# troyvvgroup/quemb

Measured on AMD Instinct MI355X. Metric: fragment CCSD iters/sec (full BE sweep over synthetic n_occ=20 n_virt=200 fragments); corr-E error vs oracle in parity_max_abs_err_Eh / parity_n220_abs_err_Eh, higher is better.
Workload: dtype f64

## Files before the change

### include/qemb_hip_ops.h

```cpp
#ifndef QEMB_HIP_OPS_H
#define QEMB_HIP_OPS_H
#include "qemb_hip.h"
#ifdef __cplusplus
extern "C" {
#endif

#define QEMB_TIMER_LADDER 0
#define QEMB_TIMER_RINGS 1
#define QEMB_TIMER_ITER 2
#define QEMB_TIMER_AO2MO 3
#define QEMB_TIMER_SCF 4
#define QEMB_TIMER_GEMM_ANY 5
#define QEMB_TIMER_SCHMIDT 6
#define QEMB_TIMER_DF 7
int qemb_timer_begin(int slot);
int qemb_timer_end(int slot);
int qemb_timer_read(int slot, double* total_ms, int64_t* count);
int qemb_timer_reset(int slot);
int qemb_alloc_stats(long long* n_driver_allocs, long long* n_driver_frees, double* ms_in_driver_calls, double* gb_allocated, int reset);
int qemb_gemm_flop_count(double* flops, int reset);
int qemb_tape_cache_counters(int64_t* reused, int64_t* recorded, int reset);
int qemb_ctx_timer_read(int ctx, int slot, double* total_ms, int64_t* count, int reset);
int qemb_timer_live_events(int slot);


int qemb_op_gemm(int64_t M, int64_t N, int64_t K, double alpha, const double* A, int64_t lda, int a_kcontig,
                 int64_t strideA, const double* B, int64_t ldb, int b_kcontig, int64_t strideB, double beta,
                 double* C, int64_t ldc, int64_t strideC, int64_t batch);
int qemb_op_gemm_slab_rows(int64_t M, int64_t N, int64_t K, const double* A, int64_t lda, int64_t a_slab, int64_t a_slab_skip, const double* B, int64_t ldb,
                           int b_kcontig, double* C, int64_t ldc, int cfg);
int qemb_set_gemm_config(int cfg);
int qemb_mfma_f64_peak(int iters, int blocks_per_cu, double* tflops);
int qemb_set_gemm_splitk(int enabled);
int qemb_op_gemm_probe(int64_t M, int64_t N, int64_t K, const double* A, int64_t lda, int a_kcontig, const double* B, int64_t ldb, int b_kcontig,
                       double* C, int64_t ldc, int cfg, int ksplit, double* ms, double* clock_ghz, int64_t* workgroups);
int qemb_op_gemm_stamps(int64_t M, int64_t N, int64_t K, const double* A, int64_t lda, const double* B, int64_t ldb, double* C, int64_t ldc, int cfg,
                        int ksplit, double* out7);
int qemb_pair_gemm_choice(int64_t rows, int64_t cols, int* cfg, int* ksplit);
int qemb_set_gemm_ksplit(int ksplit);
int qemb_op_copy4(const int64_t dim[4], const double* in, const int64_t si[4], double* out,
                  const int64_t so[4], double alpha, double beta);
int qemb_op_outer4(const int64_t dim[4], const double* u, int64_t su0, int64_t su2, const double* v,
                   int64_t sv1, int64_t sv3, double* out, const int64_t so[4], double alpha, double beta);
int qemb_op_div_denom(double* x, int64_t d0, int64_t d1, int64_t d2, int64_t d3, const double* ea,
                      const double* eb, const double* ec, const double* ed);
int qemb_op_ladder_pack_vvvv(int64_t n, int64_t o, const double* M, double* Vp, int64_t ldp, double* Vm, int64_t ldm);
int qemb_op_ladder_pack_tau(int64_t o, int64_t v, const double* tau, double* Tp, int64_t ldp, double* Tm, int64_t ldm);
int qemb_op_ladder_scatter_pm(int64_t o, int64_t v, const double* Rp, int64_t ldp, const double* Rm, int64_t ldm, double* t2);
int qemb_op_dot(int64_t n, const double* x, const double* y, double* out_dev);
int qemb_op_absmax(int64_t n, const double* x, double* out_dev);
int qemb_op_gemv_rows(int64_t rows, int64_t cols, const double* T, int64_t ldt, const double* x, double* y,
                      double alpha, double beta);
int qemb_op_gemv_rows_batched(int64_t rows, int64_t cols, int64_t nbatch, const double* T, int64_t ldt, int64_t strideT,
                              const double* x, int64_t stridex, double* y, double alpha, double beta);
int qemb_op_contract_mid(int64_t outer, int64_t mid, int64_t inner, const double* T, const double* x,
                         double* Y, int64_t ldy, double alpha, double beta);
int qemb_op_unpack_s4(int64_t n, const double* s4, double* s1);
int qemb_op_pack_s4(int64_t n, const double* s1, double* s4);
int qemb_op_unpack_s8_to_s4(int64_t n, const double* s8, double* s4);
int qemb_op_mirror_lower(int64_t n, double* A, int64_t lda);
int qemb_op_k_from_pairs(int64_t n, const double* H, const double* D, double* K);
int qemb_op_jk_from_packed(int64_t n, const double* S4, const double* D, const double* Dp, double* Jp, double* K);
int qemb_op_pack_pm_cols(int64_t rows, int64_t v, const double* in, double* Op, int64_t ldp, double* Om, int64_t ldm);
int qemb_op_scatter_pm_rows(int64_t o, int64_t ncols, const double* Xp, const double* Xm, double* out);
int qemb_op_pack_w_pm(int64_t o, const double* W, double* Ap, int64_t lda_p, double* Am, int64_t lda_m);
int qemb_op_ladder_scatter_pm2(int64_t o, int64_t v, const double* Rp, int64_t ldp, const double* Rm, int64_t ldm, const double* Hp, const double* Hm,
                               int assign, double* t2);
int qemb_op_lincomb2(int64_t n, double a, const double* x, double b, const double* y, double beta, double* out);
int qemb_op_small_k_update(int64_t batch, int64_t M, int64_t N, int64_t K, double alpha, const double* A, int64_t sA, const double* B, int64_t sB, double* C, int64_t sC);
int qemb_op_ccsd_ph_layouts(int64_t o, int64_t v, const double* t2, const double* t1, double* T, double* Tp, double* S, double* Ut, double* Tpt, double* Th);
int qemb_op_ccsd_y_traces(int64_t o, int64_t v, const double* ZC, const double* ZB, double* Y);
int qemb_op_copy4_two(const int64_t dim[4], const double* in, const int64_t si[4], double* out, const int64_t so[4], double alpha, double beta, const double* base,
                      double* out2, const double* in2, double c2a, double c2b);
int qemb_op_scatter_pm_rows_add(int64_t o, int64_t ncols, const double* Xp, const double* Xm, double* out, const double* add);
int qemb_op_ccsd_y_traces_add(int64_t o, int64_t v, const double* ZC, const double* ZB, double* Y, const double* add);
int qemb_op_pack_w_pm_sum(int64_t o, const double* Wt, const double* X, const double* At, double* Ap, int64_t lda_p, double* Am, int64_t lda_m);
int qemb_op_ccsd_t1_small(int64_t o, int64_t v, const double* t1, const double* Lvv, const double* Loo, const double* Fov, double* t1n);
int qemb_op_ccsd_t1_assemble(int64_t o, int64_t v, const double* t1, const double* Lvv, const double* Loo, const double* Fov, const double* S, const double* Lph1,
                             const double* PA, int SA, int64_t strideA, const double* PB, int SB, int64_t strideB, double* t1n);
int qemb_op_gemv_rows_two(int64_t rows1, int64_t cols1, const double* T1, int64_t ld1, const double* x1, double* y1, double a1, double b1,
                          int64_t rows2, int64_t cols2, const double* T2, int64_t ld2, const double* x2, double* y2, double a2, double b2);
int qemb_op_ccsd_y_traces_slabs(int64_t o, int64_t v, const double* ZC, const double* ZB, double* Y, const double* add, int S, int64_t stride, double scale);
int qemb_op_gemv_rows2(int64_t rows, int64_t cols, const double* T1, int64_t ld1, const double* x1, const double* T2, int64_t ld2, const double* x2, double* y, double alpha, double beta);
int qemb_op_ccsd_finish_t2_rings(int64_t o, int64_t v, double* t2n, const double* U, const double* OV, const double* RS, const double* M, const double* eo, const double* ev, double* t1n);
int qemb_op_diis_push(int64_t n, const double* trial, const double* prev, double* e, double* xcopy, int m, const double* const* ys, int self, double* row_dev, double* row_host);
int qemb_op_ccsd_extrapolate_energy(int64_t o, int64_t v, int nterms, const double* coef, const double* const* xs, double* amp, const double* L, double* tau, double* e_host);
int qemb_op_gather_rows(int64_t nrows, int64_t len, const int64_t* idx_dev, const double* src, int64_t ld, double* dst);
int qemb_op_scale_rows(int64_t nrows, int64_t len, double* x, const double* s);
int qemb_op_pack_pair_rows(int64_t n, int64_t ncols, const double* in, double* out);
int qemb_op_unpack_tril_pair_rows(int64_t nr, int64_t n, const double* in, double* full);
int qemb_op_extract_pf(int64_t n, const double* Mp, int64_t p0, int64_t q0, int64_t r0, int64_t s0, int64_t sp, int64_t sq,
                       int64_t sr, int64_t ss, double* out);
int qemb_op_extract_pf_t(int64_t n, const double* T, int64_t x0, int64_t r0, int64_t s0, int64_t c0, int64_t sx, int64_t sr,
                         int64_t ss, int64_t sc, double* out);
int qemb_op_ladder_pack_vvvv_pf(int64_t n, int64_t o, const double* Mp, double* Vp, int64_t ldp, double* Vm, int64_t ldm);
int qemb_op_unpack_tril_rows(int64_t rows, int64_t n, const double* packed, double* full);
int qemb_op_pack_tril_rows(int64_t rows, int64_t n, const double* full, double* packed);
int qemb_op_jacobi_eigh(int64_t n, double* A, double* w, double* V, int* sweeps);
int qemb_op_scf_fused_max(void);
int qemb_op_jacobi_eigh_in_basis(int64_t n, const double* F, const double* Cp, double* w, double* C_out, double* C2_out, int nocc, double* dm_out, double stop_below, int* sweeps);
int qemb_op_scf_fock_small(int64_t n, const double* h, const double* J, const double* K, const double* D, double* F, double* err, double* scal2);
int qemb_op_pack_density_sym(int64_t n, const double* D, double* Dp);
int qemb_op_jacobi_svd(int64_t m, int64_t n, double* G, double* s, double* U, double* V, int* sweeps);
int qemb_op_cholesky_lower(int64_t n, double* A);
int qemb_op_tri_inverse_lower(int64_t n, const double* L, double* Linv);


int qemb_op_mp2_amplitudes(int64_t o, int64_t v, const double* ovov, const double* eo, const double* ev, double* t2, double* G, double* e_host);

int qemb_op_rdm2_assemble(int kind, int64_t o, int64_t v, const double* t1, const double* t2, const double* dm1c, double* out);
int qemb_op_rdm2_add_nc(int64_t m, const double* g, double alpha, double* X);
int qemb_op_rdm2_symmetrize(int64_t m, const double* g, double* X);
int qemb_op_rdm2_eri_dot(int64_t m, int sym, const double* eri, const double* K, double* e_host);

int qemb_op_kdf_split(int64_t rows, int64_t nao, const double* z, double* planes);
int qemb_op_kdf_stack(int64_t nk, int64_t nao, int64_t n, const double* ta, double* Cs, double* Dk);
int qemb_op_kdf_pack(int64_t naux, int64_t n, const double* M, int paired, double w, double* F, int64_t ldf, double* out2_host);

int qemb_frag_prepare_ccsd(qemb_frag_t f, int nsocc, const double* h, const double* dm0, const qemb_solver_opts* opts);
int qemb_frag_ccsd_iterate(qemb_frag_t f, int niter, double* e_corr, double* normt);
int qemb_frag_ccsd_reset(qemb_frag_t f);
int qemb_frag_ccsd_export(qemb_frag_t f, const char* name, double* host, int64_t nelem);


int qemb_op_boys(int m_max, int64_t n, const double* x, double* out);
int qemb_op_int3c_class(int la, int lb, int lP, const void* bf_a, const void* bf_b, const void* bf_P, const double* c2s, double* out_host);
int qemb_op_int4c_class(int la, int lb, int lc, int ld, const void* bf_a, const void* bf_b, const void* bf_c, const void* bf_d, const double* c2s, double* out_host);
int qemb_op_int4c_tile(void* basis, const int32_t* pairs_r, int64_t n_r, const int32_t* pairs_s, int64_t n_s, double thresh, double* out_host);
int qemb_op_cd_panel_factor(int n, const double* A_host, double thr, double* T_host, int32_t* piv_host, int32_t* rank, int* in_lds);
int qemb_op_cd_diag_update(int64_t np, int r, const double* Lnew_host, const int32_t* pivrow_host, double* d_host, int64_t nsp, const int32_t* row0_host, const int32_t* cnt_host,
                           double* spmax_host, double* dmax_host);
int qemb_op_cd_permute(int64_t M, int64_t N, const double* L_host, const int32_t* pos_host, int full, double* out_host);
int qemb_op_df_get_ints(void* df, double* out_host, int* identity_metric);

int qemb_op_fci_sigma(int n, int nsocc, const double* h_host, const double* V_dev, const double* c_dev, double* sigma_dev);
int qemb_op_fci_rdm12(int n, int nsocc, const double* c_dev, int cumulant, double* dm1_host, double* dm2_dev);
int qemb_op_fci_sigma_timed(int n, int nsocc, const double* h_host, const double* V_dev, const double* c_dev, double* sigma_dev, double* ms3);
int qemb_op_fci_links(int n, int nsocc, int64_t* ns, int* nlink, int32_t* strings_host, int32_t* links_host);

#ifdef __cplusplus
}
#endif
#endif
```

### quemb_amd/_lib.py

```python

from __future__ import annotations

import ctypes as C
import os
from pathlib import Path

import numpy as np

_HERE = Path(__file__).resolve().parent
LIB_PATH = _HERE / "libqemb_hip.so"

c_dp = C.POINTER(C.c_double)
c_i64 = C.c_int64
c_vp = C.c_void_p


QEMB_ERR_ARG, QEMB_ERR_ALLOC, QEMB_ERR_DEVICE, QEMB_ERR_NOCONV, QEMB_ERR_NUMERIC, QEMB_ERR_UNSUPPORTED = -1, -2, -3, -4, -5, -6


class QembError(RuntimeError):

    def __init__(self, msg="", status=None):
        super().__init__(msg)
        self.status = status


class SolverOpts(C.Structure):
    _fields_ = [("struct_size", C.c_uint32), ("cc_conv_tol", C.c_double), ("cc_conv_tol_normt", C.c_double), ("cc_max_cycle", C.c_int),
                ("cc_diis_space", C.c_int), ("scf_conv_tol", C.c_double), ("scf_conv_tol_grad", C.c_double),
                ("scf_max_cycle", C.c_int), ("scf_diis_space", C.c_int), ("warm_start", C.c_int), ("verbose", C.c_int),
                ("relax_density", C.c_int), ("lambda_conv_tol", C.c_double), ("lambda_max_cycle", C.c_int),
                ("strict_convergence", C.c_int)]


class FciOpts(C.Structure):
    _fields_ = [("struct_size", C.c_uint32), ("conv_tol", C.c_double), ("max_cycle", C.c_int), ("max_space", C.c_int), ("lindep", C.c_double)]


_lib = None
_initialised_device = None


def _declare(lib):
    def f(name, restype, *argtypes):
        fn = getattr(lib, name)
        fn.restype = restype
        fn.argtypes = list(argtypes)

    I, D, P, V, L = C.c_int, C.c_double, c_vp, c_vp, c_i64
    f("qemb_init", I, I)
    f("qemb_last_error", C.c_char_p)
    f("qemb_backend", C.c_char_p)
    f("qemb_sync", I)
    f("qemb_device_sync", I)
    f("qemb_mem_info", I, C.POINTER(C.c_size_t), C.POINTER(C.c_size_t))
    f("qemb_malloc", I, C.POINTER(c_vp), C.c_size_t)
    f("qemb_free", I, V)
    f("qemb_trim", I)
    f("qemb_trim_all", I)
    f("qemb_h2d", I, V, V, C.c_size_t)
    f("qemb_d2h", I, V, V, C.c_size_t)
    f("qemb_h2d_async", I, V, V, C.c_size_t)
    f("qemb_d2d", I, V, V, C.c_size_t)
    f("qemb_timer_begin", I, I)
    f("qemb_timer_end", I, I)
    f("qemb_timer_read", I, I, C.POINTER(D), C.POINTER(L))
    f("qemb_timer_reset", I, I)
    f("qemb_timer_live_events", I, I)
    f("qemb_op_gemm", I, L, L, L, D, P, L, I, L, P, L, I, L, D, P, L, L, L)
    f("qemb_op_gemm_slab_rows", I, L, L, L, P, L, L, L, P, L, I, P, L, I)
    f("qemb_op_gemm_probe", I, L, L, L, P, L, I, P, L, I, P, L, I, I, C.POINTER(D), C.POINTER(D), C.POINTER(L))
    f("qemb_op_gemm_stamps", I, L, L, L, P, L, P, L, P, L, I, I, C.POINTER(D))
    f("qemb_set_gemm_config", I, I)
    f("qemb_set_gemm_splitk", I, I)
    f("qemb_set_gemm_ksplit", I, I)
    f("qemb_pair_gemm_choice", I, L, L, C.POINTER(I), C.POINTER(I))
    f("qemb_op_ladder_pack_vvvv", I, L, L, P, P, L, P, L)
    f("qemb_op_ladder_pack_tau", I, L, L, P, P, L, P, L)
    f("qemb_op_ladder_scatter_pm", I, L, L, P, L, P, L, P)
    f("qemb_mfma_f64_peak", I, I, I, C.POINTER(D))
    f("qemb_op_copy4", I, C.POINTER(L), P, C.POINTER(L), P, C.POINTER(L), D, D)
    f("qemb_op_outer4", I, C.POINTER(L), P, L, L, P, L, L, P, C.POINTER(L), D, D)
    f("qemb_op_div_denom", I, P, L, L, L, L, P, P, P, P)
    f("qemb_op_dot", I, L, P, P, P)
    f("qemb_op_mp2_amplitudes", I, L, L, P, P, P, P, P, C.POINTER(D))
    f("qemb_op_rdm2_assemble", I, I, L, L, P, P, P, P)
    f("qemb_op_rdm2_add_nc", I, L, P, D, P)
    f("qemb_op_rdm2_symmetrize", I, L, P, P)
    f("qemb_op_rdm2_eri_dot", I, L, I, P, P, C.POINTER(D))
    f("qemb_op_absmax", I, L, P, P)
    f("qemb_op_gemv_rows", I, L, L, P, L, P, P, D, D)
    f("qemb_op_gemv_rows_batched", I, L, L, L, P, L, L, P, L, P, D, D)
    f("qemb_op_contract_mid", I, L, L, L, P, P, P, L, D, D)
    f("qemb_op_unpack_s4", I, L, P, P)
    f("qemb_op_pack_s4", I, L, P, P)
    f("qemb_op_unpack_s8_to_s4", I, L, P, P)
    f("qemb_op_unpack_tril_rows", I, L, L, P, P)
    f("qemb_op_pack_pair_rows", I, L, L, P, P)
    f("qemb_op_mirror_lower", I, L, P, L)
    f("qemb_op_k_from_pairs", I, L, P, P, P)
    f("qemb_op_jk_from_packed", I, L, P, P, P, P, P)
    f("qemb_op_pack_pm_cols", I, L, L, P, P, L, P, L)
    f("qemb_op_scatter_pm_rows", I, L, L, P, P, P)
    f("qemb_op_pack_w_pm", I, L, P, P, L, P, L)
    f("qemb_op_ladder_scatter_pm2", I, L, L, P, L, P, L, P, P, I, P)
    f("qemb_op_lincomb2", I, L, D, P, D, P, D, P)
    f("qemb_op_small_k_update", I, L, L, L, L, D, P, L, P, L, P, L)
    f("qemb_op_ccsd_ph_layouts", I, L, L, P, P, P, P, P, P, P, P)
    f("qemb_op_ccsd_y_traces", I, L, L, P, P, P)
    f("qemb_op_copy4_two", I, C.POINTER(L), P, C.POINTER(L), P, C.POINTER(L), D, D, P, P, P, D, D)
    f("qemb_op_scatter_pm_rows_add", I, L, L, P, P, P, P)
    f("qemb_op_ccsd_y_traces_add", I, L, L, P, P, P, P)
    f("qemb_op_pack_w_pm_sum", I, L, P, P, P, P, L, P, L)
    f("qemb_op_ccsd_t1_small", I, L, L, P, P, P, P, P)
    f("qemb_op_gemv_rows2", I, L, L, P, L, P, P, L, P, P, D, D)
    f("qemb_op_ccsd_t1_assemble", I, L, L, P, P, P, P, P, P, P, I, L, P, I, L, P)
    f("qemb_op_gemv_rows_two", I, L, L, P, L, P, P, D, D, L, L, P, L, P, P, D, D)
    f("qemb_op_ccsd_y_traces_slabs", I, L, L, P, P, P, P, I, L, D)
    f("qemb_op_ccsd_finish_t2_rings", I, L, L, P, P, P, P, P, P, P, P)
    f("qemb_op_diis_push", I, L, P, P, P, P, I, P, I, P, P)
    f("qemb_op_ccsd_extrapolate_energy", I, L, L, I, P, P, P, P, P, P)
    f("qemb_op_gather_rows", I, L, L, P, P, L, P)
    f("qemb_op_scale_rows", I, L, L, P, P)
    f("qemb_ctx_count", I, I)
    f("qemb_ctx_bind", I, I)
    f("qemb_ctx_partition", I, I)
    f("qemb_ctx_timer_read", I, I, I, C.POINTER(C.c_double), C.POINTER(c_i64), I)
    f("qemb_gemm_flop_count", I, C.POINTER(C.c_double), I)
    f("qemb_tape_cache_counters", I, C.POINTER(L), C.POINTER(L), I)
    f("qemb_alloc_stats", I, C.POINTER(C.c_longlong), C.POINTER(C.c_longlong), C.POINTER(C.c_double), C.POINTER(C.c_double), I)
    f("qemb_op_unpack_tril_pair_rows", I, L, L, P, P)
    f("qemb_op_extract_pf", I, L, P, L, L, L, L, L, L, L, L, P)
    f("qemb_op_extract_pf_t", I, L, P, L, L, L, L, L, L, L, L, P)
    f("qemb_op_ladder_pack_vvvv_pf", I, L, L, P, P, L, P, L)
    f("qemb_op_pack_tril_rows", I, L, L, P, P)
    f("qemb_op_jacobi_eigh", I, L, P, P, P, C.POINTER(I))
    f("qemb_op_scf_fused_max", I)
    f("qemb_op_jacobi_eigh_in_basis", I, L, P, P, P, P, P, I, P, D, C.POINTER(I))
    f("qemb_op_scf_fock_small", I, L, P, P, P, P, P, P, P)
    f("qemb_op_pack_density_sym", I, L, P, P)
    f("qemb_op_jacobi_svd", I, L, L, P, P, P, P, C.POINTER(I))
    f("qemb_op_cholesky_lower", I, L, P)
    f("qemb_op_tri_inverse_lower", I, L, P, P)
    f("qemb_comm_unique_id", I, P)
    f("qemb_comm_init", I, I, I, P)
    f("qemb_comm_info", I, C.POINTER(I), C.POINTER(I))
    f("qemb_comm_allreduce", I, P, L, I)
    f("qemb_comm_destroy", I)
    OP = C.POINTER(SolverOpts)
    IP = C.POINTER(I)
    DP = C.POINTER(D)
    f("qemb_default_opts", None, OP)
    f("qemb_frag_create", I, I, I, C.POINTER(c_vp))
    f("qemb_frag_free", I, V)
    f("qemb_frag_set_eri_s4", I, V, P)
    f("qemb_frag_set_eri_s4_dev", I, V, P)
    f("qemb_frag_set_df_factor", I, V, I, P)
    f("qemb_frag_set_df_factor_dev", I, V, I, P)
    f("qemb_frag_mo_route", I, V, I)
    f("qemb_frag_set_df_only", I, V, I, P)
    f("qemb_frag_set_df_only_dev", I, V, I, V)
    f("qemb_frag_resident_bytes", I, V, C.POINTER(L))
    f("qemb_frag_mo_route_used", I, V, IP, IP)
    f("qemb_frag_get_eri_s4", I, V, P)
    f("qemb_frag_set_energy_data", I, V, P, P, P, D, IP, I)
    f("qemb_frag_jk", I, V, P, P, P)
    f("qemb_frag_solve", I, V, I, P, P, OP, I, P, P, P, P, P, P, P, DP, DP, DP, IP, IP)
    f("qemb_frag_solve_mp2", I, V, I, P, P, OP, I, P, P, P, P, P, P, DP, DP, DP, IP)
    f("qemb_frag_solve_mp2_batch", I, I, P, IP, P, P, OP, I, P, P, P, P, P, P, P, P, P, IP)
    f("qemb_default_fci_opts", None, C.POINTER(FciOpts))
    f("qemb_frag_solve_fci", I, V, I, P, P, OP, C.POINTER(FciOpts), I, P, P, P, P, P, P, DP, DP, DP, IP, IP)
    f("qemb_frag_fci_bytes", I, I, I, I, C.POINTER(L))
    f("qemb_frag_fci_mem_limit", I, V, L)
    f("qemb_frag_fci_residual", I, V, DP)
    f("qemb_op_fci_sigma", I, I, I, P, P, P, P)
    f("qemb_op_fci_rdm12", I, I, I, P, I, P, P)
    f("qemb_op_fci_sigma_timed", I, I, I, P, P, P, P, P)
    f("qemb_op_fci_links", I, I, I, C.POINTER(L), IP, P, P)
    f("qemb_frag_rdm2", I, V, I, I, P)
    f("qemb_frag_rdm2_mem_limit", I, V, L)
    f("qemb_frag_rdm2_dev", I, V, I, I, P)
    f("qemb_rdm2_full_guard", I, L, L, L)
    f("qemb_frag_lambda_iters", I, P, C.POINTER(C.c_int))
    f("qemb_frag_solve_batch", I, I, P, IP, P, P, OP, I, P, P, P, P, P, P, P, P, P, P, IP, IP, C.POINTER(L))
    f("qemb_frag_scf", I, V, I, P, P, OP, P, P, P, P, DP, IP, IP)
    f("qemb_frag_cphf", I, V, I, P, P, OP, P, I, P)
    f("qemb_ccsd_solve", I, I, I, I, P, P, P, OP, P, P, D, IP, I, P, P, P, P, P, P, DP, IP)
    f("qemb_frag_prepare_ccsd", I, V, I, P, P, OP)
    f("qemb_frag_ccsd_iterate", I, V, I, DP, DP)
    f("qemb_frag_ccsd_reset", I, V)
    f("qemb_frag_ccsd_export", I, V, C.c_char_p, P, L)
    LP = C.POINTER(L)
    f("qemb_aoeri_upload", I, I, P, I, C.POINTER(c_vp))
    f("qemb_aoeri_free", I, V)
    f("qemb_ao2mo_dense", I, V, P, I, P, V)
    f("qemb_df_create", I, I, P, C.POINTER(c_vp))
    f("qemb_lpq_upload", I, P, I, C.POINTER(c_vp))
    f("qemb_df_create_pbc", I, I, P, C.POINTER(c_vp), IP)
    f("qemb_df_alloc_ints", I, V, I)
    f("qemb_df_add_pw_block", I, V, I, P, P, P, P)
    f("qemb_df_add_rs_block", I, V, I, I, P)
    f("qemb_df_pw_imag_absmax", I, V, C.POINTER(C.c_double))
    f("qemb_df_pw_select", I, V, I)
    f("qemb_df_free", I, V)
    f("qemb_df_set_ints", I, V, I, P, I)
    f("qemb_df_set_ints_semisparse", I, V, I, L, P, P, P, P)
    f("qemb_df_transform", I, V, P, I, P, V)
    f("qemb_df_transform_screened", I, V, P, I, P, D, P, V)
    f("qemb_df_transform_factor", I, V, P, I, V)
    f("qemb_df_transform_screened_factor", I, V, P, I, P, D, V)
    f("qemb_kdf_create", I, I, I, I, IP, IP, C.POINTER(c_vp))
    f("qemb_kdf_set_pair", I, V, I, I, P)
    f("qemb_kdf_transform", I, V, P, I, P, V, I)
    f("qemb_kdf_free", I, V)
    f("qemb_kdf_guard", I, I, I, I, I, I, I, L)
    f("qemb_frag_get_df_factor", I, V, P)
    f("qemb_int_basis_create", I, I, P, C.c_size_t, P, C.POINTER(c_vp))
    f("qemb_int_basis_free", I, V)
    f("qemb_int3c2e", I, V, V, P, L, I, P, I)
    f("qemb_int2c2e", I, V, P, I)
    f("qemb_df_create_empty", I, C.POINTER(c_vp))
    f("qemb_df_set_ints_from_basis", I, V, V, V)
    f("qemb_df_set_ints_semisparse_from_basis", I, V, V, V, L, P, P, P, P)
    f("qemb_int4c2e", I, V, I, D, P, I)
    f("qemb_int4c_mem_limit", I, V, L)
    f("qemb_int4c_stats", I, V, C.POINTER(L), C.POINTER(L))
    f("qemb_aoeri_from_basis", I, V, D, C.POINTER(c_vp))
    f("qemb_int_jk_direct", I, V, P, D, P, P, I)
    f("qemb_int_jk_direct_bytes", I, V, C.POINTER(L))
    f("qemb_ao2mo_direct", I, V, I, P, P, P, P, L, D)
    f("qemb_ao2mo_direct_bytes", I, V, I, P, L, C.POINTER(L))
    f("qemb_int4c_tile_stats", I, V, C.POINTER(L), C.POINTER(L))
    f("qemb_op_int4c_tile", I, V, P, L, P, L, D, P)
    f("qemb_int_cholesky", I, V, D, D, L, L, P, C.POINTER(L))
    f("qemb_int_cholesky_bytes", I, V, L, L, C.POINTER(L))
    f("qemb_int_cholesky_stats", I, V, P)
    f("qemb_df_set_ints_from_cholesky", I, V, V, D, D, L, L)
    f("qemb_op_cd_panel_factor", I, I, P, D, P, P, C.POINTER(C.c_int32), C.POINTER(I))
    f("qemb_op_cd_diag_update", I, L, I, P, P, P, L, P, P, P, P)
    f("qemb_op_cd_permute", I, L, L, P, P, I, P)
    f("qemb_op_df_get_ints", I, V, P, C.POINTER(I))
    f("qemb_op_int4c_class", I, I, I, I, I, P, P, P, P, P, P)
    f("qemb_op_boys", I, I, L, P, P)
    f("qemb_op_int3c_class", I, I, I, I, P, P, P, P, P)
    f("qemb_op_kdf_split", I, L, L, P, P)
    f("qemb_op_kdf_stack", I, L, L, L, P, P, P)
    f("qemb_op_kdf_pack", I, L, L, P, I, D, P, L, DP)
    f("qemb_schmidt", I, P, I, I, I, LP, I, D, P, I, IP, IP)
    f("qemb_schmidt_subspace", I, P, I, I, I, LP, I, D, P, I, IP, IP)
    f("qemb_schmidt_svd", I, P, I, LP, I, D, P, I, IP, IP)
    f("qemb_nsocc_guess", I, P, I, I, P, IP, P)
    f("qemb_matmul", I, L, L, L, P, I, P, I, P)
    f("qemb_abs_overlap_prim", I, I, P, P, P, P, L, I, P, P, P)
    return lib


def load(path: os.PathLike | None = None):
    global _lib
    if _lib is None:
        p = Path(path) if path else LIB_PATH
        if not p.exists():
            raise QembError(
                f"{p} not found: build it with `python -c 'import __graft_entry__ as g; g.build()'` "
                "(make -C quemb_amd/csrc). quemb_amd has no CPU fallback."
            )
        _lib = _declare(C.CDLL(str(p)))
    return _lib


def declare(cdll):
    return _declare(cdll)


class ConvergenceWarning(RuntimeWarning):
    """A fragment solve did not converge and `strict_convergence = 0` asked for PySCF's behaviour (warn, carry on)."""


def check(rc: int, what: str = "", lib=None):
    if rc > 0:
        import warnings
        msg = (lib or load()).qemb_last_error().decode(errors="replace")
        warnings.warn(ConvergenceWarning(f"{what or 'libqemb_hip call'}: {msg}"), stacklevel=3)
    elif rc != 0:
        msg = (lib or load()).qemb_last_error().decode(errors="replace")
        raise QembError(f"{what or 'libqemb_hip call'} failed (status {rc}): {msg}", status=int(rc))


# ... 57 lines not shown
```

### quemb_amd/csrc/api.cpp

```cpp
#include <cstring>
#include <cstdlib>
#include <vector>
#include <execinfo.h>
#include <signal.h>
#include <unistd.h>
#include "../../include/qemb_hip_ops.h"
#include "dev_ops.h"
#include "ccsd.h"
#include "fragment.h"
#include "ao2mo.h"
#include "kdf.h"
#include "int3c.h"
#include "int4c.h"
#include "cd_core.h"
#include <mutex>
#include <set>

using namespace qemb;
namespace qemb {
int dev_mfma_f64_peak(int iters, int blocks_per_cu, double* tflops);
int schmidt_eigh(const double* lmo, int N, int nmo, int nocc, const int64_t* frag, int n_f, double thr, double* TA_out,
                 int ld_out, int* n_b_out, int* sweeps_out);
int schmidt_subspace(const double* lmo, int N, int nmo, int nocc, const int64_t* frag, int n_f, double thr, double* TA_out,
                     int ld_out, int* n_b_out, int* sweeps_out);
// ... 61 lines not shown
int qemb_set_gemm_ksplit(int ks) { g_test_ksplit = ks; return QEMB_OK; }
int qemb_set_gemm_config(int cfg) { dev_gemm_set_force_cfg(cfg); return QEMB_OK; }
#ifndef QEMB_HOSTCHECK
int qemb_mfma_f64_peak(int iters, int blocks_per_cu, double* tflops) { return dev_mfma_f64_peak(iters, blocks_per_cu, tflops); }
#else
int qemb_mfma_f64_peak(int, int, double*) { set_error("not available in the hostcheck build"); return QEMB_ERR_DEVICE; }
#endif
int qemb_pair_gemm_choice(int64_t rows, int64_t cols, int* cfg, int* ksplit) {
  int c = -1, k = 0;
  pick_pair_gemm(rows, cols, c, k);
  if (cfg) *cfg = c;
  if (ksplit) *ksplit = k;
  return QEMB_OK;
}
int qemb_set_gemm_splitk(int enabled) { dev_gemm_set_auto_splitk(enabled); return QEMB_OK; }
int qemb_op_copy4(const int64_t dim[4], const double* in, const int64_t si[4], double* out, const int64_t so[4],
                  double alpha, double beta) {
  Copy4Desc c{};
  for (int k = 0; k < 4; ++k) { c.dim[k] = dim[k]; c.si[k] = si[k]; c.so[k] = so[k]; }
  c.in = in; c.out = out; c.alpha = alpha; c.beta = beta;
  return dev_copy4(c);
}
int qemb_op_outer4(const int64_t dim[4], const double* u, int64_t su0, int64_t su2, const double* v, int64_t sv1,
                   int64_t sv3, double* out, const int64_t so[4], double alpha, double beta) {
  Outer4Desc o{};
  for (int k = 0; k < 4; ++k) { o.dim[k] = dim[k]; o.so[k] = so[k]; }
  o.u = u; o.su0 = su0; o.su2 = su2; o.v = v; o.sv1 = sv1; o.sv3 = sv3; o.out = out; o.alpha = alpha; o.beta = beta;
  return dev_outer4(o);
}
int qemb_op_div_denom(double* x, int64_t d0, int64_t d1, int64_t d2, int64_t d3, const double* ea, const double* eb,
                      const double* ec, const double* ed) { return dev_div_denom(x, d0, d1, d2, d3, ea, eb, ec, ed); }
int qemb_op_ladder_pack_vvvv(int64_t n, int64_t o, const double* M, double* Vp, int64_t ldp, double* Vm, int64_t ldm) { return dev_ladder_pack_vvvv(n, o, M, Vp, ldp, Vm, ldm); }
int qemb_op_ladder_pack_tau(int64_t o, int64_t v, const double* tau, double* Tp, int64_t ldp, double* Tm, int64_t ldm) { return dev_ladder_pack_tau(o, v, tau, Tp, ldp, Tm, ldm); }
int qemb_op_ladder_scatter_pm(int64_t o, int64_t v, const double* Rp, int64_t ldp, const double* Rm, int64_t ldm, double* t2) { return dev_ladder_scatter_pm(o, v, Rp, ldp, Rm, ldm, t2); }
int qemb_op_dot(int64_t n, const double* x, const double* y, double* o) { return dev_dot(n, x, y, o); }
int qemb_op_absmax(int64_t n, const double* x, double* o) { return dev_absmax(n, x, o); }
int qemb_op_gemv_rows(int64_t rows, int64_t cols, const double* T, int64_t ldt, const double* x, double* y, double alpha,
                      double beta) { return dev_gemv_rows(rows, cols, T, ldt, x, y, alpha, beta); }
int qemb_op_gemv_rows_batched(int64_t rows, int64_t cols, int64_t nbatch, const double* T, int64_t ldt, int64_t strideT, const double* x,
                              int64_t stridex, double* y, double alpha, double beta) { return dev_gemv_rows_batched(rows, cols, nbatch, T, ldt, strideT, x, stridex, y, alpha, beta); }
int qemb_op_contract_mid(int64_t outer, int64_t mid, int64_t inner, const double* T, const double* x, double* Y,
                         int64_t ldy, double alpha, double beta) { return dev_contract_mid(outer, mid, inner, T, x, Y, ldy, alpha, beta); }
int qemb_op_unpack_s4(int64_t n, const double* s4, double* s1) { return dev_unpack_s4(n, s4, s1); }
int qemb_op_pack_s4(int64_t n, const double* s1, double* s4) { return dev_pack_s4(n, s1, s4); }
int qemb_op_unpack_s8_to_s4(int64_t n, const double* s8, double* s4) { return dev_unpack_s8_to_s4(n, s8, s4); }
int qemb_comm_unique_id(void* id) { return dev_comm_unique_id(id); }
int qemb_comm_init(int rank, int world, const void* id) { return dev_comm_init(rank, world, id); }
int qemb_comm_info(int* rank, int* world) { return dev_comm_info(rank, world); }
int qemb_comm_allreduce(double* buf, int64_t n, int op) { return dev_comm_allreduce(buf, n, op); }
int qemb_comm_destroy(void) { return dev_comm_destroy(); }
int qemb_ctx_count(int n) { return dev_ctx_count(n); }
int qemb_ctx_bind(int k) { return dev_ctx_bind(k); }
int qemb_ctx_partition(int parts) { return dev_ctx_partition(parts); }
int qemb_op_gemm_slab_rows(int64_t M, int64_t N, int64_t K, const double* A, int64_t lda, int64_t a_slab, int64_t a_slab_skip, const double* B, int64_t ldb,
                           int b_kcontig, double* C, int64_t ldc, int cfg) {
  GemmDesc g{};
  g.M = M; g.N = N; g.K = K; g.alpha = 1.0; g.beta = 0.0;
  g.A = A; g.lda = lda; g.a_kcontig = 0; g.strideA = 0; g.a_slab = a_slab; g.a_slab_skip = a_slab_skip;
  g.B = B; g.ldb = ldb; g.b_kcontig = b_kcontig; g.strideB = 0;
  g.C = C; g.ldc = ldc; g.strideC = 0; g.batch = 1; g.cfg = cfg; g.ksplit = 0;
  return dev_gemm(g);
}
int qemb_gemm_flop_count(double* flops, int reset) { return dev_gemm_flop_count(flops, reset); }
int qemb_tape_cache_counters(int64_t* reused, int64_t* recorded, int reset) {
  long long a = 0, b = 0;
  tape_cache_counters(&a, &b, reset);
  if (reused) *reused = a;
  if (recorded) *recorded = b;
  return QEMB_OK;
}
int qemb_alloc_stats(long long* n, long long* nfree, double* ms, double* gb, int reset) { return dev_alloc_stats(n, nfree, ms, gb, reset); }
int qemb_ctx_timer_read(int ctx, int slot, double* total_ms, int64_t* count, int reset) { return dev_ctx_timer_read(ctx, slot, total_ms, count, reset); }
int qemb_op_k_from_pairs(int64_t n, const double* H, const double* D, double* K) { return dev_k_from_pairs(n, H, D, K); }
int qemb_op_jk_from_packed(int64_t n, const double* S4, const double* D, const double* Dp, double* Jp, double* K) { return dev_jk_from_packed(n, S4, D, Dp, Jp, K); }
int qemb_op_pack_pm_cols(int64_t rows, int64_t v, const double* in, double* Op, int64_t ldp, double* Om, int64_t ldm) { return dev_pack_pm_cols(rows, v, in, Op, ldp, Om, ldm); }
int qemb_op_scatter_pm_rows(int64_t o, int64_t ncols, const double* Xp, const double* Xm, double* out) { return dev_scatter_pm_rows(o, ncols, Xp, Xm, out); }
int qemb_op_pack_w_pm(int64_t o, const double* W, double* Ap, int64_t lda_p, double* Am, int64_t lda_m) { return dev_pack_w_pm(o, W, Ap, lda_p, Am, lda_m); }
int qemb_op_ladder_scatter_pm2(int64_t o, int64_t v, const double* Rp, int64_t ldp, const double* Rm, int64_t ldm, const double* Hp, const double* Hm,
                               int assign, double* t2) { return dev_ladder_scatter_pm2(o, v, Rp, ldp, Rm, ldm, Hp, Hm, assign, t2); }
int qemb_op_lincomb2(int64_t n, double a, const double* x, double b, const double* y, double beta, double* out) {
  const double c[2] = {a, b};
  const double* xs[2] = {x, y};
  return dev_lincomb(n, 2, c, xs, beta, out);
}
int qemb_op_mirror_lower(int64_t n, double* A, int64_t lda) { return dev_mirror_lower(n, A, lda); }
int qemb_op_small_k_update(int64_t batch, int64_t M, int64_t N, int64_t K, double alpha, const double* A, int64_t sA, const double* B, int64_t sB, double* C, int64_t sC) {
  return dev_small_k_update(batch, M, N, K, alpha, A, sA, B, sB, C, sC);
}
int qemb_op_ccsd_ph_layouts(int64_t o, int64_t v, const double* t2, const double* t1, double* T, double* Tp, double* S, double* Ut, double* Tpt, double* Th) {
  return dev_ccsd_ph_layouts(o, v, t2, t1, T, Tp, S, Ut, Tpt, Th);
}
int qemb_op_copy4_two(const int64_t dim[4], const double* in, const int64_t si[4], double* out, const int64_t so[4], double alpha, double beta, const double* base,
                      double* out2, const double* in2, double c2a, double c2b) {
  Copy4Desc c{};
  for (int k = 0; k < 4; ++k) { c.dim[k] = dim[k]; c.si[k] = si[k]; c.so[k] = so[k]; }
  c.in = in; c.out = out; c.alpha = alpha; c.beta = beta; c.base = base;
  c.out2 = out2; c.in2 = in2; c.c2a = c2a; c.c2b = c2b;
  return dev_copy4(c);
}
int qemb_op_scatter_pm_rows_add(int64_t o, int64_t ncols, const double* Xp, const double* Xm, double* out, const double* add) { return dev_scatter_pm_rows(o, ncols, Xp, Xm, out, add); }
int qemb_op_ccsd_y_traces_add(int64_t o, int64_t v, const double* ZC, const double* ZB, double* Y, const double* add) { return dev_ccsd_y_traces(o, v, ZC, ZB, Y, add); }
int qemb_op_pack_w_pm_sum(int64_t o, const double* Wt, const double* X, const double* At, double* Ap, int64_t lda_p, double* Am, int64_t lda_m) {
  return dev_pack_w_pm_sum(o, Wt, X, At, Ap, lda_p, Am, lda_m);
}
int qemb_op_ccsd_t1_small(int64_t o, int64_t v, const double* t1, const double* Lvv, const double* Loo, const double* Fov, double* t1n) { return dev_ccsd_t1_small(o, v, t1, Lvv, Loo, Fov, t1n); }
int qemb_op_ccsd_t1_assemble(int64_t o, int64_t v, const double* t1, const double* Lvv, const double* Loo, const double* Fov, const double* S, const double* Lph1,
                             const double* PA, int SA, int64_t strideA, const double* PB, int SB, int64_t strideB, double* t1n) {
  return dev_ccsd_t1_assemble(o, v, t1, Lvv, Loo, Fov, S, Lph1, PA, SA, strideA, PB, SB, strideB, t1n);
}
int qemb_op_gemv_rows_two(int64_t rows1, int64_t cols1, const double* T1, int64_t ld1, const double* x1, double* y1, double a1, double b1,
                          int64_t rows2, int64_t cols2, const double* T2, int64_t ld2, const double* x2, double* y2, double a2, double b2) {
  return dev_gemv_rows_two(rows1, cols1, T1, ld1, x1, y1, a1, b1, rows2, cols2, T2, ld2, x2, y2, a2, b2);
}
int qemb_op_ccsd_y_traces_slabs(int64_t o, int64_t v, const double* ZC, const double* ZB, double* Y, const double* add, int S, int64_t stride, double scale) {
  return dev_ccsd_y_traces(o, v, ZC, ZB, Y, add, S, stride, scale);
}
int qemb_op_gemv_rows2(int64_t rows, int64_t cols, const double* T1, int64_t ld1, const double* x1, const double* T2, int64_t ld2, const double* x2, double* y, double alpha, double beta) {
  return dev_gemv_rows2(rows, cols, T1, ld1, x1, T2, ld2, x2, y, alpha, beta);
}
int qemb_op_ccsd_finish_t2_rings(int64_t o, int64_t v, double* t2n, const double* U, const double* OV, const double* RS, const double* M, const double* eo, const double* ev, double* t1n) {
  return dev_ccsd_finish_t2_rings(o, v, t2n, U, OV, RS, M, eo, ev, t1n);
}
int qemb_op_diis_push(int64_t n, const double* trial, const double* prev, double* e, double* xcopy, int m, const double* const* ys, int self, double* row_dev, double* row_host) {
  void* pin = nullptr;
  QTRY(dev_pinned_alloc(&pin, sizeof(double) * 8));
  int rc = dev_diis_push(n, trial, prev, e, xcopy, m, ys, self, row_dev, (double*)pin);
  if (!rc) rc = dev_sync();
  if (!rc) for (int j = 0; j < m; ++j) row_host[j] = ((double*)pin)[j];
  dev_pinned_free(pin);
  return rc;
}
int qemb_op_ccsd_extrapolate_energy(int64_t o, int64_t v, int nterms, const double* coef, const double* const* xs, double* amp, const double* L, double* tau, double* e_host) {
  void* pin = nullptr;
  DBuf e_dev;
  QTRY(e_dev.alloc(1));
  QTRY(dev_pinned_alloc(&pin, sizeof(double) * 8));
  int rc = dev_ccsd_extrapolate_energy(o, v, nterms, coef, xs, amp, L, tau, e_dev, (double*)pin);
  if (!rc) rc = dev_sync();
  if (!rc) *e_host = *(double*)pin;
  dev_pinned_free(pin);
  return rc;
}
int qemb_op_ccsd_y_traces(int64_t o, int64_t v, const double* ZC, const double* ZB, double* Y) { return dev_ccsd_y_traces(o, v, ZC, ZB, Y); }
int qemb_op_gather_rows(int64_t nrows, int64_t len, const int64_t* idx_dev, const double* src, int64_t ld, double* dst) { return dev_gather_rows(nrows, len, idx_dev, src, ld, dst); }
int qemb_op_scale_rows(int64_t nrows, int64_t len, double* x, const double* s) { return dev_scale_rows(nrows, len, x, s); }
int qemb_op_pack_pair_rows(int64_t n, int64_t ncols, const double* in, double* out) { return dev_pack_pair_rows(n, ncols, in, out); }
int qemb_op_extract_pf(int64_t n, const double* Mp, int64_t p0, int64_t q0, int64_t r0, int64_t s0, int64_t sp, int64_t sq, int64_t sr, int64_t ss, double* out) {
  return dev_extract_pf(n, Mp, p0, q0, r0, s0, sp, sq, sr, ss, out);
}
int qemb_op_extract_pf_t(int64_t n, const double* T, int64_t x0, int64_t r0, int64_t s0, int64_t c0, int64_t sx, int64_t sr, int64_t ss, int64_t sc, double* out) {
  return dev_extract_pf_t(n, T, x0, r0, s0, c0, sx, sr, ss, sc, out);
}
int qemb_op_ladder_pack_vvvv_pf(int64_t n, int64_t o, const double* Mp, double* Vp, int64_t ldp, double* Vm, int64_t ldm) { return dev_ladder_pack_vvvv_pf(n, o, Mp, Vp, ldp, Vm, ldm); }
int qemb_op_unpack_tril_pair_rows(int64_t nr, int64_t n, const double* in, double* full) { return dev_unpack_tril_pair_rows(nr, n, in, full); }
int qemb_op_unpack_tril_rows(int64_t rows, int64_t n, const double* p, double* f) { return dev_unpack_tril_rows(rows, n, p, f); }
int qemb_op_pack_tril_rows(int64_t rows, int64_t n, const double* f, double* p) { return dev_pack_tril_rows(rows, n, f, p); }
int qemb_op_jacobi_eigh(int64_t n, double* A, double* w, double* V, int* sweeps) { return dev_jacobi_eigh(n, A, w, V, sweeps); }
int qemb_op_scf_fused_max(void) { return dev_scf_fused_max(); }
int qemb_op_jacobi_eigh_in_basis(int64_t n, const double* F, const double* Cp, double* w, double* C_out, double* C2_out, int nocc, double* dm_out, double stop_below, int* sweeps) {
  DBuf st;
  QTRY(st.alloc(1));
  QTRY(dev_jacobi_eigh_in_basis(n, F, Cp, w, C_out, C2_out, nocc, dm_out, stop_below, reinterpret_cast<int*>(st.p)));
  double word = 0.0;
  QTRY(dev_d2h(&word, st.p, sizeof(double)));
  int sw; std::memcpy(&sw, &word, sizeof(int));
  if (sweeps) *sweeps = sw;
  if (sw < 0) { set_error("Jacobi sweeps did not converge in 40 sweeps"); return QEMB_ERR_NOCONV; }
  return QEMB_OK;
}
int qemb_op_scf_fock_small(int64_t n, const double* h, const double* J, const double* K, const double* D, double* F, double* err, double* scal2) { return dev_scf_fock_small(n, h, J, K, D, F, err, scal2); }
int qemb_op_pack_density_sym(int64_t n, const double* D, double* Dp) { return dev_pack_density_sym(n, D, Dp); }
int qemb_op_jacobi_svd(int64_t m, int64_t n, double* G, double* s, double* U, double* V, int* sweeps) { return dev_jacobi_svd(m, n, G, s, U, V, sweeps); }
int qemb_op_cholesky_lower(int64_t n, double* A) { return dev_cholesky_lower(n, A); }
int qemb_op_tri_inverse_lower(int64_t n, const double* L, double* Linv) { return dev_tri_inverse_lower(n, L, Linv); }
int qemb_op_boys(int m_max, int64_t n, const double* x, double* out) { QTRY(dev_boys(m_max, n, x, out)); return dev_sync(); }
int qemb_op_int4c_class(int la, int lb, int lc, int ld, const void* bf_a, const void* bf_b, const void* bf_c, const void* bf_d, const double* c2s, double* out_host) {
  const int l[4] = {la, lb, lc, ld};
  const BfRecord* const rec[4] = {reinterpret_cast<const BfRecord*>(bf_a), reinterpret_cast<const BfRecord*>(bf_b), reinterpret_cast<const BfRecord*>(bf_c), reinterpret_cast<const BfRecord*>(bf_d)};
  return int4c_block(l, rec, c2s, out_host);
}
int qemb_op_int3c_class(int la, int lb, int lP, const void* bf_a, const void* bf_b, const void* bf_P, const double* c2s, double* out_host) {
  return int3c_block(la, lb, lP, reinterpret_cast<const BfRecord*>(bf_a), reinterpret_cast<const BfRecord*>(bf_b), reinterpret_cast<const BfRecord*>(bf_P), c2s, out_host);
}
int qemb_op_mp2_amplitudes(int64_t o, int64_t v, const double* ovov, const double* eo, const double* ev, double* t2, double* G, double* e_host) {
  DBuf part, e;
  QTRY(part.alloc(dev_mp2_partial_count(o, v))); QTRY(e.alloc(1));
  QTRY(dev_mp2_amplitudes(o, v, ovov, eo, ev, t2, G, part, e));
  return e_host ? dev_d2h(e_host, e, sizeof(double)) : dev_sync();
}

int qemb_op_rdm2_assemble(int kind, int64_t o, int64_t v, const double* t1, const double* t2, const double* dm1c, double* out) {
  QTRY(dev_rdm2_assemble(kind, o, v, t1, t2, dm1c, out));
  return dev_sync();
}

int qemb_op_rdm2_add_nc(int64_t m, const double* g, double alpha, double* X) { return dev_rdm2_add_nc(m, g, alpha, X); }
int qemb_op_rdm2_symmetrize(int64_t m, const double* g, double* X) { return dev_rdm2_symmetrize(m, g, X); }
int qemb_op_rdm2_eri_dot(int64_t m, int sym, const double* eri, const double* K, double* e_host) {
  if (!e_host) { set_error("qemb_op_rdm2_eri_dot: e_host is NULL"); return QEMB_ERR_ARG; }
  DBuf w;
  QTRY(w.alloc(rdm2_full_grid(m > 0 ? m : 1) + 1));
  QTRY(dev_rdm2_eri_dot(m, sym, eri, K, w.p + 1, w.p));
  return dev_d2h(e_host, w.p, sizeof(double));
}

int qemb_op_kdf_split(int64_t rows, int64_t nao, const double* z, double* planes) { QTRY(dev_kdf_split(rows, nao, z, planes)); return dev_sync(); }
int qemb_op_kdf_stack(int64_t nk, int64_t nao, int64_t n, const double* ta, double* Cs, double* Dk) { QTRY(dev_kdf_stack(nk, nao, n, ta, Cs, Dk)); return dev_sync(); }
int qemb_op_kdf_pack(int64_t naux, int64_t n, const double* M, int paired, double w, double* F, int64_t ldf, double* out2_host) {
  if (!out2_host) { set_error("qemb_op_kdf_pack: out2_host is NULL"); return QEMB_ERR_ARG; }
  DBuf wk;
  QTRY(wk.alloc(dev_kdf_partial_count(naux > 0 ? naux : 1, n > 0 ? n : 1) + 2));
  QTRY(dev_kdf_pack(naux, n, M, paired, w, F, ldf, wk.p + 2, wk.p));
  return dev_d2h(out2_host, wk.p, 2 * sizeof(double));
}

void qemb_default_opts(qemb_solver_opts* o) {
  CcsdOptions c; ScfOptions s;
  memset(o, 0, sizeof *o);
  o->struct_size = (uint32_t)sizeof(qemb_solver_opts);
  o->cc_conv_tol = c.conv_tol; o->cc_conv_tol_normt = c.conv_tol_normt; o->cc_max_cycle = c.max_cycle; o->cc_diis_space = c.diis_space;
  o->scf_conv_tol = s.conv_tol; o->scf_conv_tol_grad = s.conv_tol_grad; o->scf_max_cycle = s.max_cycle; o->scf_diis_space = s.diis_space;
  o->warm_start = 0; o->verbose = 0;
  LambdaOptions l;
  o->relax_density = 0; o->lambda_conv_tol = l.conv_tol; o->lambda_max_cycle = l.max_cycle;
  o->strict_convergence = 1;
}
static FragmentOptions to_opts(const qemb_solver_opts* o) {
  FragmentOptions f;
  if (o) {
    f.cc.conv_tol = o->cc_conv_tol; f.cc.conv_tol_normt = o->cc_conv_tol_normt; f.cc.max_cycle = o->cc_max_cycle;
    f.cc.diis_space = o->cc_diis_space; f.cc.verbose = o->verbose;
    f.scf.conv_tol = o->scf_conv_tol; f.scf.conv_tol_grad = o->scf_conv_tol_grad; f.scf.max_cycle = o->scf_max_cycle;
    f.scf.diis_space = o->scf_diis_space; f.scf.verbose = o->verbose;
    f.warm_start = o->warm_start;
    f.relax_density = o->relax_density; f.lam.conv_tol = o->lambda_conv_tol; f.lam.max_cycle = o->lambda_max_cycle;
    f.lam.diis_space = o->cc_diis_space; f.lam.verbose = o->verbose;
    f.strict = o->strict_convergence;
  }
  return f;
}
#define CHECK_OPTS(o)                                                                                                     \
  do {                                                                                                                    \
    if ((o) && (o)->struct_size != (uint32_t)sizeof(qemb_solver_opts)) {                                                  \
      set_error("qemb_solver_opts.struct_size is " + std::to_string((o)->struct_size) + ", this library expects " +       \
                std::to_string(sizeof(qemb_solver_opts)) + ": initialise the struct with qemb_default_opts() (binding built " \
                "against another qemb_hip.h?)");                                                                          \
      return QEMB_ERR_ARG;                                                                                                \
    }                                                                                                                     \
  } while (0)
#define FRAG(f) (reinterpret_cast<Fragment*>(f))
#define CHECK_FRAG(f) do { if (!(f)) { set_error("null fragment handle"); return QEMB_ERR_ARG; } } while (0)

int qemb_frag_create(int n, int n_f, qemb_frag_t* out) {
  if (n <= 0 || n_f < 0 || n_f > n || !out) { set_error("qemb_frag_create: bad arguments"); return QEMB_ERR_ARG; }
  *out = new Fragment(n, n_f);
  return QEMB_OK;
}
int qemb_frag_free(qemb_frag_t f) { delete FRAG(f); return QEMB_OK; }
int qemb_frag_set_eri_s4(qemb_frag_t f, const double* s4) { CHECK_FRAG(f); return FRAG(f)->set_eri_s4_host(s4); }
int qemb_frag_set_eri_s4_dev(qemb_frag_t f, const double* s4) { CHECK_FRAG(f); return FRAG(f)->set_eri_s4_dev(s4); }
int qemb_frag_set_df_factor(qemb_frag_t f, int naux, const double* B) { CHECK_FRAG(f); return FRAG(f)->set_df_factor_host(naux, B); }
int qemb_frag_set_df_factor_dev(qemb_frag_t f, int naux, const double* B) { CHECK_FRAG(f); return FRAG(f)->set_df_factor_dev(naux, B); }
int qemb_frag_set_df_only(qemb_frag_t f, int naux, const double* B) { CHECK_FRAG(f); return FRAG(f)->set_df_only_host(naux, B); }
int qemb_frag_set_df_only_dev(qemb_frag_t f, int naux, const double* B) { CHECK_FRAG(f); return FRAG(f)->set_df_only_dev(naux, B); }
int qemb_frag_resident_bytes(qemb_frag_t f, int64_t* bytes) { CHECK_FRAG(f); if (!bytes) { set_error("qemb_frag_resident_bytes: null argument"); return QEMB_ERR_ARG; } *bytes = FRAG(f)->resident_bytes(); return QEMB_OK; }
int qemb_frag_mo_route(qemb_frag_t f, int route) { CHECK_FRAG(f); return FRAG(f)->set_mo_route(route); }
int qemb_frag_mo_route_used(qemb_frag_t f, int* used_factor, int* naux) {
  CHECK_FRAG(f);
  if (used_factor) *used_factor = FRAG(f)->last_route_was_factor() ? 1 : 0;
  if (naux) *naux = FRAG(f)->df_naux();
  return QEMB_OK;
}
int qemb_frag_get_eri_s4(qemb_frag_t f, double* s4) {
  CHECK_FRAG(f);
  if (!s4) { set_error("qemb_frag_get_eri_s4: null buffer"); return QEMB_ERR_ARG; }
  return FRAG(f)->export_eri_s4(s4);
}
int qemb_frag_get_df_factor(qemb_frag_t f, double* B) {
  CHECK_FRAG(f);
  if (!B) { set_error("qemb_frag_get_df_factor: null buffer"); return QEMB_ERR_ARG; }
  return FRAG(f)->export_df_factor(B);
}
int qemb_frag_set_energy_data(qemb_frag_t f, const double* h1, const double* veff0, const double* veff, double weight,
                              const int* centers, int ncenter) {
  CHECK_FRAG(f);
  for (int i = 0; i < ncenter; ++i) if (centers[i] < 0 || centers[i] >= FRAG(f)->nf()) { set_error("centre index outside the fragment sites"); return QEMB_ERR_ARG; }
  FRAG(f)->set_energy_data(h1, veff0, veff, weight, centers, ncenter);
  return QEMB_OK;
}
int qemb_frag_jk(qemb_frag_t f, const double* P, double* J, double* K) { CHECK_FRAG(f); return FRAG(f)->hf_veff_from_dm(P, J, K); }
int qemb_frag_solve(qemb_frag_t f, int nsocc, const double* h, const double* dm0, const qemb_solver_opts* opts, int eeval,
                    double* mo_coeff, double* mo_energy, double* rdm1_emb, double* rdm1_mo, double* t1, double* t2,
                    double* e_frag, double* e_corr_mo, double* e_scf, double* ebe_hf, int* n_iter, int* scf_cycles) {
  CHECK_FRAG(f); CHECK_OPTS(opts);
  if (!h) { set_error("qemb_frag_solve: h is NULL"); return QEMB_ERR_ARG; }
  FragmentResult r;
  int rc = FRAG(f)->solve(nsocc, h, dm0, to_opts(opts), eeval, &r, mo_coeff, mo_energy, rdm1_emb, rdm1_mo, t1, t2);
  if (n_iter) *n_iter = r.n_iter;
  if (scf_cycles) *scf_cycles = r.scf_cycles;
  FRAG(f)->last_lambda_iters = r.lambda_iters;
  if (rc < 0) return rc;
  if (e_frag) { e_frag[0] = r.e_frag[0]; e_frag[1] = r.e_frag[1]; e_frag[2] = r.e_frag[2]; }
  if (e_corr_mo) *e_corr_mo = r.e_corr_mo;
  if (e_scf) *e_scf = r.e_scf;
  if (ebe_hf) *ebe_hf = r.ebe_hf;
  return rc;
// ... 665 lines not shown
```

### quemb_amd/csrc/ccsd.cpp

```cpp
#include "ccsd.h"
#include "ao2mo.h"
#include <algorithm>
#include <chrono>
#include <cmath>
#include <cstdio>
#include <cstdlib>
#include <cstring>
#include <string>

namespace qemb {

int mo_slab_ld(int n) { return (n >= 64 && n <= 1024) ? (n + 15) / 16 * 16 : n; }
int64_t mo_transform_work(int n) { return (int64_t)n * mo_slab_ld(n) * ((int64_t)n * (n + 1) / 2); }

static int mo_three_quarter_blocks(int n, int o, int nf, const double* T, int64_t slab, MoIntegrals& out, bool build_T34) {
  const int v = n - o;
  if (nf > 0 && build_T34) {
    QTRY(out.T34.alloc((int64_t)n * n * n * nf));
    QTRY(dev_extract_pf_t(n, T, 0, 0, 0, 0, n, n, n, nf, out.T34, slab));
  } else if (nf > 0) {
    QTRY(out.A1.alloc((int64_t)v * o * v * nf));
    QTRY(out.A2.alloc((int64_t)o * o * v * nf));
    QTRY(dev_extract_pf_t(n, T, o, 0, o, 0, v, o, v, nf, out.A1, slab));
    QTRY(dev_extract_pf_t(n, T, 0, 0, o, 0, o, o, v, nf, out.A2, slab));
  }
  return 0;
}

static int mo_blocks_from_pair_first(int n, int o, const double* Mp, double* scratch, int64_t scratch_elems, MoIntegrals& out, bool build_Vl) {
  const int v = n - o;
  QTRY(out.oooo.alloc((int64_t)o * o * o * o));
  QTRY(out.ovoo.alloc((int64_t)o * v * o * o));
  QTRY(out.ovov.alloc((int64_t)o * v * o * v));
  QTRY(out.oovv.alloc((int64_t)o * o * v * v));
  QTRY(out.ovvo.alloc((int64_t)o * v * v * o));
  QTRY(out.ovvv.alloc((int64_t)o * v * v * v));
  QTRY(dev_extract_pf(n, Mp, 0, 0, 0, 0, o, o, o, o, out.oooo));
  QTRY(dev_extract_pf(n, Mp, 0, o, 0, 0, o, v, o, o, out.ovoo));
  QTRY(dev_extract_pf(n, Mp, 0, o, 0, o, o, v, o, v, out.ovov));
  QTRY(dev_extract_pf(n, Mp, 0, 0, o, o, o, o, v, v, out.oovv));
  QTRY(dev_extract_pf(n, Mp, 0, o, o, 0, o, v, v, o, out.ovvo));
  QTRY(dev_extract_pf(n, Mp, 0, o, o, o, o, v, v, v, out.ovvv));
  {
    const int64_t npv = (int64_t)v * (v + 1) / 2, nm = (int64_t)v * (v - 1) / 2;
    out.ldp = npv + (npv & 1); out.ldm = nm + (nm & 1);
    if (out.ldm == 0) out.ldm = 2;
    QTRY(out.Vp.alloc(npv * out.ldp));
    QTRY(out.Vm.alloc(std::max<int64_t>(nm, 1) * out.ldm));
    QTRY(dev_ladder_pack_vvvv_pf(n, o, Mp, out.Vp, out.ldp, out.Vm, out.ldm));
  }
  if (build_Vl) {
    const int64_t v4 = (int64_t)v * v * v * v;
    QTRY(out.Vl.alloc(v4));
    DBuf tmp;
    double* g = scratch;
    if (!g || v4 > scratch_elems) { QTRY(tmp.alloc(v4)); g = tmp; }
    QTRY(dev_extract_pf(n, Mp, o, o, o, o, v, v, v, v, g));
    QTRY(perm4(out.Vl, g, v, v, v, v, 0, 2, 1, 3));
  }
  return 0;
}

int mo_transform(int n, int o, int nf, const double* eri_s4, double* X0, double* X1, const double* C, MoIntegrals& out, bool build_Vl, bool build_T34,
                 bool x1_is_unpacked) {
  const int v = n - o;
  const int64_t np = (int64_t)n * (n + 1) / 2, ncol = np * n;
  out.n = n; out.o = o; out.v = v; out.nf = nf;
  TimerScope lap_AO2MO(TIMER_AO2MO);
  const int64_t nl = mo_slab_ld(n);
  if (!x1_is_unpacked) QTRY(dev_unpack_tril_rows_ld(np, n, nl, eri_s4, X1));
  const int tcfg = (n > 192 && n <= 224) ? 13 : -1;
  QTRY(gemm(n, ncol, n, 1.0, C, n, false, X1, nl, true, 0.0, X0, ncol, 1, 0, 0, 0, tcfg));
  QTRY(gemm_quarter_lower_rows(n, np, n, C, X0, X1));
  QTRY(dev_unpack_tril_pair_rows_ld(n, n, nl, X1, X0));
  const int64_t n2 = (int64_t)n * n;
  if (n > 192 && n <= 224) { QTRY(gemm(np * n, n, n, 1.0, X0, nl, true, C, n, false, 0.0, X1, n, 1, 0, 0, 0, 34)); }
  else QTRY(gemm(n, n, n, 1.0, X0, nl, true, C, n, false, 0.0, X1, n, np, (int64_t)n * nl, 0, n2, tcfg));
  QTRY(mo_three_quarter_blocks(n, o, nf, X1, 0, out, build_T34));
  if (n > 192 && n <= 224 && n % 2 == 0) {
    GemmDesc g{};
    g.M = np * n; g.N = n; g.K = n; g.alpha = 1.0; g.beta = 0.0;
    g.A = X1; g.lda = n; g.a_kcontig = 0; g.strideA = 0; g.a_slab = n; g.a_slab_skip = n2 - n;
    g.B = C; g.ldb = n; g.b_kcontig = 0; g.strideB = 0;
    g.C = X0; g.ldc = n; g.strideC = 0; g.batch = 1; g.cfg = 34; g.ksplit = 0;
    QTRY(dev_gemm(g));
  } else QTRY(gemm(n, n, n, 1.0, C, n, false, X1, n, false, 0.0, X0, n, np, 0, n2, n2, tcfg));
  QTRY(mo_blocks_from_pair_first(n, o, X0, X1, mo_transform_work(n), out, build_Vl));
  QTRY(lap_AO2MO.close());
  return 0;
}

int mo_transform_factor(int n, int o, int nf, int naux, const double* Bf, double* X0, double* X1, const double* C, MoIntegrals& out, bool build_Vl,
                        bool build_T34) {
  const int v = n - o;
  const int64_t np = (int64_t)n * (n + 1) / 2, n2 = (int64_t)n * n;
  if (naux <= 0 || !Bf) { set_error("mo_transform_factor: no factor"); return QEMB_ERR_ARG; }
  if ((int64_t)nf * n > mo_transform_work(n) / np) { set_error("mo_transform_factor: work buffer too small"); return QEMB_ERR_ARG; }
  out.n = n; out.o = o; out.v = v; out.nf = nf;
  TimerScope lap_AO2MO(TIMER_AO2MO);
  DBuf Lu, Lh, Lpk;
  QTRY(Lu.alloc((int64_t)naux * n2)); QTRY(Lh.alloc((int64_t)naux * n2)); QTRY(Lpk.alloc((int64_t)naux * np));
  QTRY(dev_unpack_tril_rows(naux, n, Bf, Lu));
  QTRY(gemm((int64_t)naux * n, n, n, 1.0, Lu, n, true, C, n, false, 0.0, Lh, n));
  QTRY(gemm(n, n, n, 1.0, C, n, false, Lh, n, false, 0.0, Lu, n, naux, 0, n2, n2));
  QTRY(dev_pack_tril_rows(naux, n, Lu, Lpk));
  Lu.release();
  QTRY(df_pair_product(np, naux, Lpk, X1));
  QTRY(dev_unpack_tril_rows(np, n, X1, X0));
  if (nf > 0) {
    QTRY(gemm(np, (int64_t)nf * n, naux, 1.0, Lpk, np, false, Lh, n2, false, 0.0, X1, (int64_t)nf * n));
    QTRY(mo_three_quarter_blocks(n, o, nf, X1, (int64_t)nf * n, out, build_T34));
  }
  Lh.release(); Lpk.release();
  QTRY(mo_blocks_from_pair_first(n, o, X0, X1, mo_transform_work(n), out, build_Vl));
  QTRY(lap_AO2MO.close());
  return 0;
}

static void pick_xw_split(int64_t rows, int64_t oo, int64_t K, int& cfg, int& ks);
static void pick_long_k(int64_t M, int64_t N, int64_t K, int tile_m, int tile_n, int cfg_in, int& cfg, int& ks, bool many_slices);
int CcsdSolver::setup(MoIntegrals&& ints, const double* mo_energy_dev) {
  I_ = std::move(ints);
  o_ = I_.o; v_ = I_.v; nf_ = I_.nf;
  const int64_t o = o_, v = v_, nov = o * v, oo = o * o, vv = v * v, N2 = oo * vv;
  QTRY(eo_.alloc(o)); QTRY(ev_.alloc(v));
  QTRY(dev_d2d(eo_, mo_energy_dev, sizeof(double) * o));
  QTRY(dev_d2d(ev_, mo_energy_dev + o, sizeof(double) * v));
  QTRY(ovov_t_.alloc(nov * nov)); QTRY(Lovov_.alloc(nov * nov)); QTRY(Loovv_.alloc(N2)); QTRY(OVoovv_.alloc(N2));
  QTRY(Lovoo_.alloc(o * v * oo)); QTRY(W1base_.alloc(N2)); QTRY(W2base_.alloc(N2)); QTRY(Lph1_.alloc(N2));
  QTRY(oooo_p_.alloc(oo * oo));
  QTRY(perm4(ovov_t_, I_.ovov, o, v, o, v, 0, 3, 2, 1));
  QTRY(dcopy(nov * nov, I_.ovov, Lovov_));
  QTRY(axpby(nov * nov, -1.0, ovov_t_, 2.0, Lovov_));
  QTRY(perm4(Loovv_, Lovov_, o, v, o, v, 0, 2, 1, 3));
  QTRY(perm4(OVoovv_, I_.ovov, o, v, o, v, 0, 2, 1, 3));
  QTRY(perm4(Lovoo_, I_.ovoo, o, v, o, o, 2, 1, 0, 3, -1.0, 0.0));
  QTRY(axpby(o * v * oo, 2.0, I_.ovoo, 1.0, Lovoo_));
  QTRY(LovooT_.alloc(o * v * oo));
  QTRY(perm4(LovooT_, Lovoo_, o, v, o, o, 2, 3, 0, 1));
  QTRY(ovoo_ijka_.alloc(o * v * oo));
  QTRY(perm4(ovoo_ijka_, I_.ovoo, o, v, o, o, 0, 2, 3, 1));
  QTRY(ovoo_kilc_.alloc(o * v * oo));
  QTRY(perm4(ovoo_kilc_, I_.ovoo, o, v, o, o, 2, 3, 0, 1));
  QTRY(perm4(W1base_, I_.ovvo, o, v, v, o, 3, 2, 0, 1));
  QTRY(perm4(W2base_, I_.oovv, o, o, v, v, 1, 2, 0, 3));
  QTRY(dcopy(N2, W2base_, Lph1_));
  QTRY(axpby(N2, 2.0, W1base_, -1.0, Lph1_));
  {
    DBuf OVl;
    QTRY(OVl.alloc(o * v * vv));
    QTRY(perm4(OVl, I_.ovvv, o, v, v, v, 0, 2, 3, 1));
    QTRY(OVp_.alloc(nov * I_.ldp)); QTRY(OVm_.alloc(nov * I_.ldm));
    QTRY(dev_pack_pm_cols(nov, v, OVl, OVp_, I_.ldp, OVm_, I_.ldm));
  }
  {
    const int64_t npv = v * (v + 1) / 2;
    QTRY(ovvv_pk_.alloc(o * v * npv)); QTRY(ZCp_.alloc(oo * npv));
    QTRY(dev_pack_tril_rows(o * v, v, I_.ovvv, ovvv_pk_));
  }
  QTRY(Gp_.alloc(oo * I_.ldp)); QTRY(Gm_.alloc(oo * I_.ldm));
  QTRY(dev_pack_pm_cols(oo, v, OVoovv_, Gp_, I_.ldp, Gm_, I_.ldm));
  QTRY(perm4(oooo_p_, I_.oooo, o, o, o, o, 1, 3, 0, 2));
  QTRY(ovoo_cikl_.alloc(v * oo * o));
  QTRY(perm4(ovoo_cikl_, I_.ovoo, o, v, o, o, 1, 3, 2, 0));
  const int64_t na = nov + N2;
  QTRY(amp_.alloc(na)); QTRY(ampn_.alloc(na)); QTRY(diff_.alloc(na));
  for (DBuf* b : {&tau_, &T_, &Tp_, &S_, &W1_, &W2_, &W12_, &W12b_, &R_, &U_}) QTRY(b->alloc(N2));
  const int64_t NG = std::max<int64_t>(N2, oo * o * v);
  QTRY(G2_.alloc(NG));
  {
    int cfg, ks;
    pick_long_k(v, v, oo * v, 64, 64, (v <= 256) ? 1 : -1, cfg, ks, false);
    QTRY(Fvv_.alloc((int64_t)gemm_slab_count(oo * v, ks) * vv));
    const int cw = (o <= 32) ? 21 : -1;
    pick_long_k(o, v, o * vv, 32, 128, cw, cfg, ks, true);
    const int64_t sa = gemm_slab_count(o * vv, ks);
    pick_long_k(o, v, o * v * o, 32, 128, cw, cfg, ks, true);
    const int64_t sb = gemm_slab_count(o * v * o, ks);
    QTRY(T1P_.alloc((sa + sb) * nov));
  }
  QTRY(Foo_.alloc(oo)); QTRY(Fov_.alloc(nov)); QTRY(Z_.alloc(oo)); QTRY(Y_.alloc(vv));
  QTRY(Ytmp_.alloc(vv)); QTRY(Loo_.alloc(oo)); QTRY(Lvv_.alloc(vv)); QTRY(Q_.alloc(oo)); QTRY(Wo_.alloc(oo * oo));
  QTRY(O1_.alloc(oo * oo)); QTRY(X_.alloc(oo * nov)); QTRY(scal_.alloc(8));
  {
    const int64_t npo = o * (o + 1) / 2, nmo = std::max<int64_t>(o * (o - 1) / 2, 1);
    const int64_t npv = v * (v + 1) / 2, nmv = v * (v - 1) / 2;
    auto slabs_pair = [&](int64_t rows, int64_t cols, int64_t K, bool k_aware = false) { int cfg, ks; pick_pair_gemm(rows, cols, cfg, ks, k_aware ? K : 0); return (int64_t)gemm_slab_count(K, ks); };
    auto slabs_xw = [&](int64_t rows, int64_t K) { int cfg, ks; pick_xw_split(rows, oo, K, cfg, ks); return (int64_t)gemm_slab_count(K, ks); };
    QTRY(LTp_.alloc(npo * I_.ldp)); QTRY(LRp_.alloc(std::max(npo * I_.ldp, slabs_pair(npo, npv, I_.ldp) * npo * npv)));
    QTRY(LTm_.alloc(nmo * I_.ldm)); QTRY(LRm_.alloc(std::max(nmo * I_.ldm, slabs_pair(nmo, std::max<int64_t>(nmv, 1), I_.ldm) * nmo * std::max<int64_t>(nmv, 1))));
    QTRY(Xp_.alloc(slabs_pair(npo, nov, I_.ldp, true) * npo * nov)); QTRY(Xm_.alloc(slabs_pair(nmo, nov, I_.ldm, true) * nmo * nov));
    QTRY(Xwp_.alloc(slabs_xw(npo, I_.ldp) * npo * oo)); QTRY(Xwm_.alloc(slabs_xw(nmo, I_.ldm) * nmo * oo)); QTRY(Xw_.alloc(oo * oo));
    lwp_ = npo + (npo & 1); lwm_ = std::max<int64_t>(2, nmo + (nmo & 1));
    QTRY(WAp_.alloc(npo * lwp_)); QTRY(WAm_.alloc(nmo * lwm_)); QTRY(HRp_.alloc(npo * I_.ldp)); QTRY(HRm_.alloc(nmo * I_.ldm));
    QTRY(ZB_.alloc(N2)); QTRY(ZC_.alloc(N2));
  }
  first_ = true;
  return 0;
}

int CcsdSolver::make_tau(const double* t1, const double* t2, double* tau) {
  const int64_t o = o_, v = v_;
  Outer4Desc d{};
  d.dim[0] = o; d.dim[1] = o; d.dim[2] = v; d.dim[3] = v;
  d.u = t1; d.su0 = v; d.su2 = 1; d.v = t1; d.sv1 = v; d.sv3 = 1;
  d.out = tau; d.so[0] = o * v * v; d.so[1] = v * v; d.so[2] = v; d.so[3] = 1;
  d.alpha = 1.0; d.beta = 1.0; d.base = t2;
  return dev_outer4(d);
}

int CcsdSolver::energy(const double* t1, const double* t2, double* e) {
  QTRY(make_tau(t1, t2, tau_));
  QTRY(dev_dot((int64_t)o_ * o_ * v_ * v_, Loovv_, tau_, scal_));
  if (e) QTRY(dev_d2h(e, scal_, sizeof(double)));
  return 0;
}
int CcsdSolver::fetch_energy() { return dev_d2h(&ecc_, scal_, sizeof(double)); }

int CcsdSolver::init_amps(bool defer_energy) {
  const int64_t o = o_, v = v_;
  QTRY(dev_fill(t1(), o * v, 0.0));
  QTRY(dcopy(o * o * v * v, OVoovv_, t2()));
  QTRY(dev_div_denom(t2(), o, o, v, v, eo_, eo_, ev_, ev_));
  first_ = true;
  diis_.clear();
  return energy(t1(), t2(), defer_energy ? nullptr : &ecc_);
}

int CcsdSolver::set_amps(const double* t1d, const double* t2d, bool defer_energy) {
  QTRY(dev_d2d(t1(), t1d, sizeof(double) * o_ * v_));
  QTRY(dev_d2d(t2(), t2d, sizeof(double) * (int64_t)o_ * o_ * v_ * v_));
  first_ = true;
  diis_.clear();
  return energy(t1(), t2(), defer_energy ? nullptr : &ecc_);
}

void pick_pair_gemm(int64_t rows, int64_t cols, int& cfg, int& ks, int64_t K) {
  cfg = -1; ks = 0;
  if (cols < 1024) return;
  static const struct { int rows, cfg, cols; double cost; } cand[] = {{224, 13, 128, 1.0}, {192, 15, 128, 1.0}, {160, 35, 128, 1.03}, {128, 4, 256, 1.0},
                                                                      {112, 11, 128, 1.25}, {80, 36, 128, 1.08}, {64, 12, 128, 1.6}, {48, 38, 128, 1.12}};
  double best_cost = -1.0;
  int64_t tiles = 0;
  for (const auto& c : cand) {
    const int64_t mt = (rows + c.rows - 1) / c.rows;
    if (c.cfg == 38 && mt > 1) continue;
    const double cost = (double)(mt * c.rows) * c.cost;
    if (best_cost < 0 || cost < best_cost - 1e-9) { best_cost = cost; cfg = c.cfg; tiles = mt * ((cols + c.cols - 1) / c.cols); }
  }
  double best = 0.0;
  for (int c = 1; c <= 8; ++c) {
    const int64_t units = tiles * c, rounds = (units + 255) / 256;
    const double eff = (double)units / (double)(rounds * 256) - (c == 1 ? 0.0 : 0.002 * c);
    if (units >= 512 && eff > best + 1e-9) { best = eff; ks = c; }
  }
  if (ks == 0) ks = (int)std::max<int64_t>(1, std::min<int64_t>(8, (1024 + tiles - 1) / tiles));
  if (K > 0 && tiles * ks < 256) ks = (int)std::max<int64_t>(ks, std::min<int64_t>(std::min<int64_t>(32, K / 256), (512 + tiles - 1) / tiles));
}

struct SlabGemm { int S = 1; int64_t stride = 0, ld = 0; };
static int gemm_slabs(int64_t M, int64_t N, int64_t K, const double* A, int64_t lda, const double* B, int64_t ldb, double* C, int64_t ldc, int cfg, int ks, SlabGemm& out,
                      bool a_kc = true, bool b_kc = true) {
  GemmDesc g{};
  g.M = M; g.N = N; g.K = K; g.alpha = 1.0; g.beta = 0.0;
  g.A = A; g.lda = lda; g.a_kcontig = a_kc ? 1 : 0; g.B = B; g.ldb = ldb; g.b_kcontig = b_kc ? 1 : 0;
  g.C = C; g.ldc = ldc; g.batch = 1; g.cfg = cfg; g.ksplit = ks;
  out.S = gemm_slab_count(K, ks);
  if (out.S > 1) { g.keep_slabs = 1; out.stride = M * N; out.ld = N; }
  else { out.stride = 0; out.ld = ldc; }
  return dev_gemm(g);
}
static void pick_xw_split(int64_t rows, int64_t oo, int64_t K, int& cfg, int& ks) {
  cfg = -1; ks = 0;
  if (K < 2048) return;
  const int64_t tiles = ((rows + 63) / 64) * ((oo + 63) / 64);
  cfg = 1;
  ks = (int)std::max<int64_t>(1, std::min<int64_t>(std::min<int64_t>(64, K / 256), (512 + tiles - 1) / tiles));
}
static int auto_ksplit(int64_t tiles, int64_t K) {
  if (tiles >= 256 || K < 1024) return 0;
  int64_t S = (768 + tiles - 1) / tiles;
  if (S > K / 256) S = K / 256;
  return S > 1 ? (int)S : 0;
}
static void pick_long_k(int64_t M, int64_t N, int64_t K, int tile_m, int tile_n, int cfg_in, int& cfg, int& ks, bool many_slices = false) {
  cfg = cfg_in; ks = 0;
  if (cfg_in < 0) return;
  ks = auto_ksplit(((M + tile_m - 1) / tile_m) * ((N + tile_n - 1) / tile_n), K);
  if (many_slices && ks > 1 && M <= 32 && N <= 32) ks = (int)std::min<int64_t>(512, K / 64);
}
int CcsdSolver::apply_ladder(const double* x, double* out, bool rows_packed, bool hh) {
  const int64_t o = o_, v = v_;
  {
    const int64_t npo = o * (o + 1) / 2, nmo = o * (o - 1) / 2, npv = v * (v + 1) / 2, nmv = v * (v - 1) / 2;
    const int64_t ldp = I_.ldp, ldm = I_.ldm;
    if (!rows_packed) QTRY(dev_ladder_pack_tau(o, v, x, LTp_, ldp, LTm_, ldm));
    int cfg, ks;
    TimerScope lap_LADDER(TIMER_LADDER);
    SlabGemm sp, sm;
    pick_pair_gemm(npo, npv, cfg, ks);
    if (cfg == 13 || cfg == 15) cfg += 10;
    QTRY(dev_region_begin());
    QTRY(gemm_slabs(npo, npv, ldp, LTp_, ldp, I_.Vp, ldp, LRp_, ldp, cfg, ks, sp));
    QTRY(dev_region_chain());
    if (nmo > 0 && nmv > 0) {
      pick_pair_gemm(nmo, nmv, cfg, ks);
      if (cfg == 13 || cfg == 15) cfg += 10;
      QTRY(gemm_slabs(nmo, nmv, ldm, LTm_, ldm, I_.Vm, ldm, LRm_, ldm, cfg, ks, sm));
    }
    QTRY(dev_region_end());
    QTRY(lap_LADDER.close());
// ... 445 lines not shown
```

### quemb_amd/csrc/ccsd.h

```cpp
#pragma once
#include <cstdint>
#include <vector>
#include "dev_ops.h"
#include "tensor_utils.h"

namespace qemb {

struct CcsdOptions {
  double conv_tol = 1e-10;
  double conv_tol_normt = 1e-8;
  int max_cycle = 100;
  int diis_space = 6;
  int verbose = 0;
};

struct MoIntegrals {
  int n = 0, o = 0, v = 0, nf = 0;
  DBuf oooo, ovoo, ovov, oovv, ovvo, ovvv;
  DBuf Vl;
  DBuf Vp, Vm;
  int64_t ldp = 0, ldm = 0;
  DBuf A1, A2;
  DBuf T34;
};

int mo_slab_ld(int n);
int64_t mo_transform_work(int n);
int mo_transform(int n, int o, int nf, const double* eri_s4, double* X0, double* X1, const double* C, MoIntegrals& out,
                 bool build_Vl = false, bool build_T34 = false, bool x1_is_unpacked = false);
int mo_transform_factor(int n, int o, int nf, int naux, const double* B_packed, double* X0, double* X1, const double* C, MoIntegrals& out,
                        bool build_Vl = false, bool build_T34 = false);
inline bool mo_factor_route_pays(int n, int naux) { return naux > 0 && (int64_t)naux <= 8 * (int64_t)n; }

class CcLambda;

struct LockstepStats { long long merged_runs = 0, launches = 0, grouped = 0, operations = 0, max_group = 0; double ms_tapes = 0.0, ms_post = 0.0; };
class CcsdSolver;
int ccsd_kernel_lockstep(const std::vector<CcsdSolver*>& s, const std::vector<CcsdOptions>& opt, const std::vector<int>& ctx, int home_ctx,
                         std::vector<double>& e_corr, std::vector<int>& n_iter, std::vector<char>& converged, LockstepStats* stats);

class CcsdSolver {
  friend class CcLambda;
  friend int ccsd_kernel_lockstep(const std::vector<CcsdSolver*>&, const std::vector<CcsdOptions>&, const std::vector<int>&, int,
                                  std::vector<double>&, std::vector<int>&, std::vector<char>&, LockstepStats*);
 public:
  int setup(MoIntegrals&& ints, const double* mo_energy_dev);
  int init_amps(bool defer_energy = false);
  int set_amps(const double* t1_dev, const double* t2_dev, bool defer_energy = false);
  int fetch_energy();
  int iterate(double* e_corr, double* normt);
  int iterate_update(bool prefer_tape, bool defer_tape, bool* deferred);
  int iterate_post(double* e_corr, double* normt);
  bool fused_post() const;
  int post_wait(int step);
  int post_issue();
  int post_extrapolate(double* normt);
  int post_energy(double* e_corr);
  int prepare_tape(int peers = 1);
  int kernel(const CcsdOptions& opt, double* e_corr, int* n_iter, bool* converged);
  int energy_intermediates(std::vector<double>& Z1, std::vector<double>& Z2);
  int export_block(const char* name, double* host, int64_t nelem);
  int apply_ladder(const double* x, double* out, bool rows_packed = false, bool hh = false);
  const MoIntegrals& integrals() const { return I_; }
  double* t1() { return amp_.p; }
  double* t2() { return amp_.p + (int64_t)o_ * v_; }
  int o() const { return o_; }
  int v() const { return v_; }
  int64_t n_amp() const { return (int64_t)o_ * v_ + (int64_t)o_ * o_ * v_ * v_; }

 private:
  int update_amps(double* t1n, double* t2n);
  int energy(const double* t1, const double* t2, double* e);
  int make_tau(const double* t1, const double* t2, double* tau);

  int o_ = 0, v_ = 0, nf_ = 0;
  MoIntegrals I_;
  DBuf eo_, ev_;
  DBuf ovov_t_, Lovov_, Loovv_, OVoovv_, Lovoo_, ovoo_ijka_, ovoo_kilc_, W1base_, W2base_, Lph1_, OVp_, OVm_, oooo_p_, ovoo_cikl_;
  DBuf amp_, ampn_, diff_;
  DBuf tau_, T_, Tp_, S_, W1_, W2_, W12_, W12b_, R_, U_, G2_, T1P_;
  DBuf LTp_, LTm_, LRp_, LRm_;
  DBuf Xp_, Xm_;
  DBuf ovvv_pk_, ZCp_;
  DBuf Gp_, Gm_;
  DBuf Xwp_, Xwm_, Xw_;
  DBuf WAp_, WAm_, HRp_, HRm_;
  int64_t lwp_ = 0, lwm_ = 0;
  DBuf ZB_, ZC_;
  DBuf Foo_, Fvv_, Fov_, Z_, Y_, Ytmp_, Loo_, Lvv_, Q_, Wo_, O1_, X_, scal_, LovooT_;
  std::vector<DeviceDIIS> diis_;
  bool first_ = true;
  dev_graph_t graph_ = nullptr;
  dev_tape_t tape_ = nullptr;
  int eager_iters_ = 0;
  bool graph_ok_ = true;
  double* last_out_ = nullptr;
  double* host_scal_ = nullptr;
  unsigned long long seq_push_ = 0, seq_energy_ = 0;
  bool post_pending_ = false;
  bool last_use_diis_ = false, last_replayable_ = false;
 public:
  ~CcsdSolver() {
    if (graph_) dev_graph_destroy(graph_);
    if (tape_) dev_tape_destroy(tape_);
    if (host_scal_) { if (post_pending_) (void)dev_sync_device(); dev_pinned_free(host_scal_); }
  }
  CcsdSolver() = default;
  dev_tape_t release_tape() { dev_tape_t t = tape_; tape_ = nullptr; return t; }
  void adopt_tape(dev_tape_t t) { if (tape_) dev_tape_destroy(tape_); tape_ = t; }
  dev_tape_t tape() const { return tape_; }
  CcsdSolver(const CcsdSolver&) = delete;
  CcsdSolver& operator=(const CcsdSolver&) = delete;
 private:
  double ecc_ = 0.0;
};

void pick_pair_gemm(int64_t rows, int64_t cols, int& cfg, int& ks, int64_t K = 0);
}
```

### quemb_amd/csrc/dev_ops.h

```cpp
#pragma once
#include <cstddef>
#include <cstdint>
#include <string>
#include "../../include/qemb_hip_ops.h"

namespace qemb {

void set_error(const std::string& msg);
const char* last_error();

#define QTRY(expr)              \
  do {                          \
    int _rc = (expr);           \
    if (_rc != 0) return _rc;   \
  } while (0)


int dev_init(int device);
int dev_sync();
int dev_sync_device();
int dev_ctx_count(int n);
int dev_ctx_bind(int k);
int dev_ctx_partition(int parts);
int dev_alloc(void** p, size_t bytes);
int dev_free(void* p);
int dev_trim();
int dev_trim_all();
int dev_h2d(void* dst, const void* src_host, size_t bytes);
int dev_h2d_async(void* dst, const void* src, size_t bytes);
int dev_d2h(void* dst_host, const void* src, size_t bytes);
int dev_d2h_async(void* dst_pinned, const void* src, size_t bytes);
int dev_pinned_alloc(void** p, size_t bytes);
int dev_pinned_free(void* p);
int dev_d2d(void* dst, const void* src, size_t bytes);
int dev_fill(double* x, int64_t n, double value);
int dev_mem_info(size_t* free_b, size_t* total_b);
int dev_alloc_stats(long long* n_driver_allocs, long long* n_driver_frees, double* ms_in_driver_calls, double* gb_allocated, int reset);
const char* dev_backend_name();

typedef void* dev_graph_t;
int dev_graph_begin(int for_tape = 0);
int dev_region_begin();
int dev_region_chain();
int dev_region_end();
int dev_graph_end(dev_graph_t* out);
int dev_graph_launch(dev_graph_t g);
int dev_graph_destroy(dev_graph_t g);
bool dev_capturing();
typedef void* dev_tape_t;
int dev_tape_end(dev_tape_t* out);
int dev_tape_run(const dev_tape_t* tapes, int n);
int dev_tape_destroy(dev_tape_t t);
int dev_tape_equal(dev_tape_t a, dev_tape_t b);
void dev_alloc_trace_begin();
unsigned long long dev_alloc_trace_end();
int dev_tape_last_stats(long long* launches, long long* grouped, long long* operations);

int dev_timer_begin(int slot);
int dev_timer_end(int slot);
int dev_timer_read(int slot, double* total_ms, int64_t* count);
int dev_timer_reset(int slot);
int dev_ctx_timer_read(int ctx, int slot, double* total_ms, int64_t* count, int reset);
int dev_timer_live_events(int slot);
enum { TIMER_LADDER = 0, TIMER_RINGS = 1, TIMER_ITER = 2, TIMER_AO2MO = 3, TIMER_SCF = 4,
       TIMER_GEMM_ANY = 5, TIMER_SCHMIDT = 6, TIMER_DF = 7, TIMER_NSLOTS = 16 };
struct TimerScope {
  int slot; bool open;
  explicit TimerScope(int s) : slot(s), open(dev_timer_begin(s) == 0) {}
  int close() { if (!open) return 0; open = false; return dev_timer_end(slot); }
  ~TimerScope() { if (open) (void)dev_timer_end(slot); }
  TimerScope(const TimerScope&) = delete;
  TimerScope& operator=(const TimerScope&) = delete;
};

struct GemmDesc {
  int64_t M, N, K;
  double alpha, beta;
  const double* A; int64_t lda; int a_kcontig; int64_t strideA;
  const double* B; int64_t ldb; int b_kcontig; int64_t strideB;
  double* C; int64_t ldc; int64_t strideC;
  int64_t batch;
  int cfg = -1;
  int ksplit = 0;
  int keep_slabs = 0;
  int64_t a_slab = 0, a_slab_skip = 0;
};
inline int gemm_slab_count(int64_t K, int ksplit) {
  if (ksplit <= 1) return 1;
  int64_t chunk = (K + ksplit - 1) / ksplit;
  chunk = (chunk + 31) / 32 * 32;
  const int64_t S = (K + chunk - 1) / chunk;
  return S > 1 ? (int)S : 1;
}
int dev_gemm(const GemmDesc& g);
int dev_gemm_flop_count(double* flops, int reset);
void dev_gemm_set_force_cfg(int cfg);
void dev_gemm_set_auto_splitk(int enabled);
void dev_gemm_set_peers(int n);
int dev_gemm_peers();
int dev_gemm_probe(const GemmDesc& g, double* ms, double* ghz, long long* workgroups);
int dev_gemm_stamps(const GemmDesc& g, int waves_per_wg, double* out7);

struct Copy4Desc {
  int64_t dim[4];
  const double* in; int64_t si[4];
  double* out; int64_t so[4];
  double alpha, beta;
  const double* base = nullptr;
  double* out2 = nullptr; const double* in2 = nullptr; double c2a = 0.0, c2b = 0.0;
};
int dev_copy4(const Copy4Desc& c);

struct Outer4Desc {
  int64_t dim[4];
  const double* u; int64_t su0, su2;
  const double* v; int64_t sv1, sv3;
  double* out; int64_t so[4];
  double alpha, beta;
  const double* base = nullptr;
};
int dev_outer4(const Outer4Desc& c);
int dev_lincomb(int64_t n, int nterms, const double* coef, const double* const* xs, double beta, double* out);

int dev_div_denom(double* x, int64_t d0, int64_t d1, int64_t d2, int64_t d3,
                  const double* ea, const double* eb, const double* ec, const double* ed);

int dev_mirror_lower(int64_t n, double* A, int64_t lda);

int dev_k_from_pairs(int64_t n, const double* H, const double* D, double* K);
int dev_jk_from_packed(int64_t n, const double* S4, const double* D, const double* Dp, double* Jp, double* K);

int dev_pack_pair_rows(int64_t n, int64_t ncols, const double* in, double* out);
int dev_extract_pf(int64_t n, const double* Mp, int64_t p0, int64_t q0, int64_t r0, int64_t s0, int64_t sp, int64_t sq,
                   int64_t sr, int64_t ss, double* out);
int dev_extract_pf_t(int64_t n, const double* T, int64_t x0, int64_t r0, int64_t s0, int64_t c0, int64_t sx, int64_t sr,
                     int64_t ss, int64_t sc, double* out, int64_t slab = 0);
int dev_ladder_pack_vvvv_pf(int64_t n, int64_t o, const double* Mp, double* Vp, int64_t ldp, double* Vm, int64_t ldm);

int dev_ladder_pack_vvvv(int64_t n, int64_t o, const double* M, double* Vp, int64_t ldp, double* Vm, int64_t ldm);
int dev_ladder_pack_tau(int64_t o, int64_t v, const double* tau, double* Tp, int64_t ldp, double* Tm, int64_t ldm);
int dev_pack_pm_cols(int64_t rows, int64_t v, const double* in, double* Op, int64_t ldp, double* Om, int64_t ldm);
int dev_scatter_pm_rows(int64_t o, int64_t ncols, const double* Xp, const double* Xm, double* out, const double* add = nullptr, int Sp = 1, int64_t strideP = 0,
                        int Sm = 1, int64_t strideM = 0);
int dev_ccsd_finish_t2(int64_t o, int64_t v, double* t2n, const double* U, const double* OV, const double* eo, const double* ev);
int dev_ccsd_finish_t2_rings(int64_t o, int64_t v, double* t2n, const double* U, const double* OV, const double* RS, const double* M, const double* eo, const double* ev, double* t1n);
int dev_ladder_scatter_pm(int64_t o, int64_t v, const double* Rp, int64_t ldp, const double* Rm, int64_t ldm, double* t2);
int dev_ladder_scatter_pm2(int64_t o, int64_t v, const double* Rp, int64_t ldp, const double* Rm, int64_t ldm, const double* Hp, const double* Hm,
                           int assign, double* t2, int Sp = 1, int64_t strideP = 0, int Sm = 1, int64_t strideM = 0, int64_t ldhp = 0, int64_t ldhm = 0);
int dev_pack_w_pm(int64_t o, const double* W, double* Ap, int64_t lda_p, double* Am, int64_t lda_m);
int dev_pack_w_pm_sum(int64_t o, const double* Wt, const double* X, const double* At, double* Ap, int64_t lda_p, double* Am, int64_t lda_m);
int dev_ccsd_t1_small(int64_t o, int64_t v, const double* t1, const double* Lvv, const double* Loo, const double* Fov, double* t1n);
int dev_ccsd_t1_assemble(int64_t o, int64_t v, const double* t1, const double* Lvv, const double* Loo, const double* Fov, const double* S, const double* Lph1,
                         const double* PA, int SA, int64_t strideA, const double* PB, int SB, int64_t strideB, double* t1n);
int dev_gemv_rows_two(int64_t rows1, int64_t cols1, const double* T1, int64_t ld1, const double* x1, double* y1, double a1, double b1,
                      int64_t rows2, int64_t cols2, const double* T2, int64_t ld2, const double* x2, double* y2, double a2, double b2);
int dev_gemv_rows2(int64_t rows, int64_t cols, const double* T1, int64_t ld1, const double* x1, const double* T2, int64_t ld2, const double* x2, double* y, double alpha, double beta);
int dev_foo_from_x(int64_t o, const double* X, double* F);
int dev_ccsd_ph_layouts(int64_t o, int64_t v, const double* t2, const double* t1, double* T, double* Tp, double* S, double* Ut, double* Tpt, double* Th);
int dev_small_k_update(int64_t batch, int64_t M, int64_t N, int64_t K, double alpha, const double* A, int64_t sA, const double* B, int64_t sB,
                       double* C, int64_t sC);
int dev_ccsd_y_traces(int64_t o, int64_t v, const double* ZC, const double* ZB, double* Y, const double* add = nullptr, int S = 1, int64_t stride = 0, double scale = 1.0);

inline int64_t dev_mp2_partial_count(int64_t o, int64_t v) {
  const int64_t nt = (v + 31) / 32, oo = o * o;
  return nt * (nt + 1) / 2 * (oo < 4096 ? oo : 4096);
}
int dev_mp2_amplitudes(int64_t o, int64_t v, const double* ovov, const double* eo, const double* ev, double* t2, double* G, double* partials, double* e_dev);

inline int rdm2_check_args(int kind, int64_t o, int64_t v, const double* t1, const double* t2, const double* out) {
  if (kind != QEMB_RDM2_CCSD && kind != QEMB_RDM2_MP2) { set_error("dev_rdm2_assemble: kind must be QEMB_RDM2_CCSD or QEMB_RDM2_MP2"); return QEMB_ERR_ARG; }
  if (o <= 0 || v < 0 || !out || (v > 0 && (!t2 || (kind == QEMB_RDM2_CCSD && !t1)))) { set_error("dev_rdm2_assemble: bad arguments"); return QEMB_ERR_ARG; }
  if (o + v > 32767) { set_error("dev_rdm2_assemble: n = " + std::to_string(o + v) + " is beyond any n^4 tensor"); return QEMB_ERR_ARG; }
  return 0;
}
int dev_rdm2_assemble(int kind, int64_t o, int64_t v, const double* t1, const double* t2, const double* dm1c, double* out);
inline int64_t rdm2_full_grid(int64_t m) { return m * m < 4096 ? m * m : 4096; }
inline int rdm2_check_full(int64_t m, const void* a, const void* b) {
  if (m <= 0 || m > 32767 || !a || !b) { set_error("rdm2 full-basis pass: bad arguments (N = " + std::to_string(m) + ")"); return QEMB_ERR_ARG; }
  return 0;
}
int dev_rdm2_add_nc(int64_t m, const double* g, double alpha, double* X);
int dev_rdm2_symmetrize(int64_t m, const double* g, double* X);
int dev_rdm2_eri_dot(int64_t m, int sym, const double* eri, const double* K, double* partials, double* out_dev);

constexpr int kFciMaxOrb = 16;
constexpr int64_t kFciMaxDet = (int64_t)12870 * 12870;
inline int fci_check_args(const char* who, int n, int64_t ns, int nlink, const void* a, const void* b, const void* c) {
  if (n <= 0 || n > kFciMaxOrb || ns <= 0 || ns > 12870 || nlink <= 0 || nlink > kFciMaxOrb * kFciMaxOrb || !a || !b || !c) {
    set_error(std::string(who) + ": bad arguments (n = " + std::to_string(n) + ", strings = " + std::to_string(ns) + ")");
    return QEMB_ERR_ARG;
  }
  return 0;
}
int dev_fci_gather(int n, int64_t ns, int nlink, const int32_t* links, const double* c, double* D);
int dev_fci_sigma(int n, int64_t ns, int nlink, const int32_t* links, const double* k, const double* D, const double* G, double* sigma);
int dev_fci_diag(int n, int64_t ns, const int32_t* strings, const double* h, const double* V, double* hdiag);
int dev_fci_precond(int64_t N, const double* r, const double* hdiag, double theta, double* out);
int dev_fci_dm2(int n, int o_cum, const double* A, const double* dm1, double* out);

inline int64_t kdf_ld(int64_t nao) { return (nao + 15) / 16 * 16; }
int dev_kdf_split(int64_t rows, int64_t nao, const double* z, double* planes);
int dev_kdf_stack(int64_t nk, int64_t nao, int64_t n, const double* ta, double* Cs, double* Dk);
inline int64_t dev_kdf_partial_count(int64_t naux, int64_t n) {
  const int64_t nt = (n + 31) / 32;
  return 2 * (nt * (nt + 1) / 2) * (naux < 1024 ? naux : 1024);
}
inline int kdf_check_pack(int64_t naux, int64_t n, const void* M, const void* F, int64_t ldf, const void* partials, const void* out2) {
  if (naux <= 0 || n <= 0 || n > 32767 || !M || !F || !partials || !out2 || ldf < n * (n + 1) / 2) { set_error("dev_kdf_pack: bad arguments"); return QEMB_ERR_ARG; }
  return 0;
}
int dev_kdf_pack(int64_t naux, int64_t n, const double* M, int paired, double w, double* F, int64_t ldf, double* partials, double* out2_dev);

int dev_boys(int m_max, int64_t n, const double* x, double* out);
namespace int3c { struct ClassArgs; }
int dev_int3c_class(int la, int lb, int lp, const int3c::ClassArgs& args);

namespace int4c { struct PairArgs; struct ClassArgs; }
int dev_int4c_pairs(int la, int lb, const int4c::PairArgs& args);
int dev_int4c_class(int la, int lb, int lc, int ld, const int4c::ClassArgs& args);
namespace int4c { struct JkArgs; }
namespace int3c { struct Shell; }
int dev_int4c_jk_class(int la, int lb, int lc, int ld, const int4c::JkArgs& args);
int dev_int4c_dmax(const int3c::Shell* sh, int nshell, int64_t N, const double* dm, double* out);
namespace int4c { struct PairProdArgs; }
int dev_int4c_pairprod(const int4c::PairProdArgs& args);
int dev_int4c_add_transpose(int64_t m, double* A);

int dev_cd_gather_cols(int64_t rows, int64_t ncols, const double* in, int64_t ldi, const int32_t* idx, double* out, int64_t ldo);
int dev_cd_panel_factor(const double* E, int64_t ld, const int32_t* srow, int n, double thr, const double* d, double* T, int32_t* piv, int32_t* rank, double* work);
int dev_cd_new_rows(int64_t np, int n, int r, const double* E, int64_t ld, const double* T, const int32_t* piv, double* Lnew, int64_t ldl);
int dev_cd_diag_update(int64_t np, int r, const double* Lnew, int64_t ldl, const int32_t* piv, const int32_t* srow, double* d, int64_t nsp, const int32_t* row0, const int32_t* cnt,
                       double* spmax, double* partials, double* dmax);
int dev_cd_unpack(int64_t M, int64_t N, const double* L, int64_t ld, const int32_t* pos, double* out);

int dev_threshold_mask(int64_t n, const double* x, double eps, double* out);
int dev_mul_bcast_rows(int64_t rows, int64_t cols, double* x, const double* m);

int dev_abs_overlap_prim(int nsh, const int* l, const double* ex, const double* xyz, const int64_t* cart0, int64_t ncart, int nroots,
                         const double* roots, const double* weights, double* out);

int dev_gather_rows(int64_t nrows, int64_t len, const int64_t* idx_dev, const double* src, int64_t ld, double* dst);
int dev_scale_rows(int64_t nrows, int64_t len, double* x, const double* s);

int dev_dot(int64_t n, const double* x, const double* y, double* out_dev);
int dev_absmax(int64_t n, const double* x, double* out_dev);
int dev_dot_many(int64_t n, const double* x, int m, const double* const* ys, double* out_dev);
int dev_diis_push(int64_t n, const double* trial, const double* prev, double* e, double* xcopy, int m, const double* const* ys, int self,
                  double* row_dev, double* row_host, void* flag_host = nullptr, unsigned long long seq = 0);
int dev_batch_begin();
int dev_batch_flush();
int dev_wait_flag(const void* flag_host, unsigned long long seq);
int dev_ccsd_extrapolate_energy(int64_t o, int64_t v, int nterms, const double* coef, const double* const* xs, double* amp, const double* L,
                                double* tau, double* e_dev, double* e_host, void* flag_host = nullptr, unsigned long long seq = 0);

int dev_gemv_rows(int64_t rows, int64_t cols, const double* T, int64_t ldt, const double* x,
                  double* y, double alpha, double beta);
int dev_gemv_rows_batched(int64_t rows, int64_t cols, int64_t nbatch, const double* T, int64_t ldt, int64_t strideT,
                          const double* x, int64_t stridex, double* y, double alpha, double beta);
int dev_contract_mid(int64_t outer, int64_t mid, int64_t inner, const double* T, const double* x,
                     double* Y, int64_t ldy, double alpha, double beta);

int dev_unpack_s4(int64_t n, const double* s4, double* s1);
int dev_pack_s4(int64_t n, const double* s1, double* s4);
int dev_unpack_s8_to_s4(int64_t n, const double* s8, double* s4);
int dev_unpack_tril_rows(int64_t rows, int64_t n, const double* packed, double* full);
int dev_unpack_tril_rows_ld(int64_t rows, int64_t n, int64_t ld, const double* packed, double* full);
int dev_pack_tril_rows(int64_t rows, int64_t n, const double* full, double* packed);
int dev_unpack_tril_pair_rows(int64_t nr, int64_t n, const double* in, double* full);
int dev_unpack_tril_pair_rows_ld(int64_t nr, int64_t n, int64_t ld, const double* in, double* full);

int dev_jacobi_eigh(int64_t n, double* A, double* w, double* V, int* sweeps_out);
int dev_jacobi_eigh_until(int64_t n, double* A, double* w, double* V, int* sweeps_out, double stop_below);
int dev_scf_fused_max();
int dev_jacobi_eigh_in_basis(int64_t n, const double* F, const double* Cp, double* w, double* C_out, double* C2_out, int nocc, double* dm_out, double stop_below,
                             int* status_dev);
int dev_scf_fock_small(int64_t n, const double* h, const double* J, const double* K, const double* D, double* F, double* err, double* scal2);
int dev_pack_density_sym(int64_t n, const double* D, double* Dp);
int dev_jacobi_svd(int64_t m, int64_t n, double* G, double* s, double* U, double* V, int* sweeps_out);

enum { COMM_ID_BYTES = 128, COMM_SUM = 0, COMM_MAX = 1 };
int dev_comm_unique_id(void* id128);
int dev_comm_init(int rank, int world, const void* id128);
int dev_comm_info(int* rank, int* world);
int dev_comm_allreduce(double* host_buf, int64_t n, int op);
int dev_comm_destroy();

int dev_cholesky_lower(int64_t n, double* A);
int dev_tri_inverse_lower(int64_t n, const double* L, double* Linv);

}
```

### quemb_amd/csrc/dev_ops_hip.hip

```cpp
#include <hip/hip_runtime.h>
#include <chrono>
#include <atomic>
#include <algorithm>
#include <cstdint>
#include <cstdlib>
#include <cstring>
#include <map>
#include <thread>
#include <mutex>
#include <string>
#include <type_traits>
#include <vector>
#include "dev_ops.h"
#include "hip_common.h"
#include "grouped_launch.h"

namespace qemb {
static thread_local std::string g_err;
void set_error(const std::string& msg) { g_err = msg; }
const char* last_error() { return g_err.c_str(); }

struct TimerLap { hipEvent_t e0, e1; bool ended; };
struct TimerSlot { double total_ms = 0; int64_t count = 0; std::vector<TimerLap> pending; std::vector<std::pair<hipEvent_t, hipEvent_t>> spare; };
static constexpr size_t TIMER_MAX_PENDING = 64;
// ... 1224 lines not shown
__device__ __forceinline__ void ccsd_y_traces_kernel_body(const uint3 BID, const uint3 GDIM, long long o, long long v, const double* __restrict__ ZC, const double* __restrict__ ZB,
                                                            double* __restrict__ Y, const double* __restrict__ add, int S, long long stride, double scale) {
  const long long idx = ((long long)BID.x * blockDim.x + threadIdx.x) >> 3;
  const int q = threadIdx.x & 7;
  const bool in = idx < v * v;
  const long long a = in ? idx / v : 0, c = in ? idx % v : 0;
  double s = 0.0;
  if (in) {
    double zc[4], zb[4];
    long long k = q;
    for (; k + 24 < o; k += 32) {
#pragma unroll
      for (int u = 0; u < 4; ++u) { const long long kk = k + 8 * u; zc[u] = ZC[((kk * o + kk) * v + a) * v + c]; zb[u] = ZB[((kk * v + c) * v + a) * o + kk]; }
#pragma unroll
      for (int u = 0; u < 4; ++u) s += 2.0 * zc[u] - zb[u];
    }
    for (; k < o; k += 8) s += 2.0 * ZC[((k * o + k) * v + a) * v + c] - ZB[((k * v + c) * v + a) * o + k];
  }
  s += __shfl_xor(s, 1); s += __shfl_xor(s, 2); s += __shfl_xor(s, 4);
  if (in && q == 0) Y[idx] = add ? s + scale * slab_sum(add + idx, S, stride) : s;
}
__global__ void __launch_bounds__(256) ccsd_y_traces_kernel(long long o, long long v, const double* __restrict__ ZC, const double* __restrict__ ZB,
                                                            double* __restrict__ Y, const double* __restrict__ add, int S, long long stride, double scale) { ccsd_y_traces_kernel_body(block_id(), grid_dim(), o, v, ZC, ZB, Y, add, S, stride, scale); }
static const Groupable<ccsd_y_traces_kernel_body, 256> reg_ccsd_y_traces(ccsd_y_traces_kernel);
int dev_ccsd_y_traces(int64_t o, int64_t v, const double* ZC, const double* ZB, double* Y, const double* add, int S, int64_t stride, double scale) {
  REQUIRE_INIT();
  if (v <= 0) return QEMB_OK;
  return launch("dev_ccsd_y_traces", ccsd_y_traces_kernel, dim3((unsigned)((v * v * 8 + 255) / 256)), dim3(256), 0, g_stream, o, v, ZC, ZB, Y, add, std::max(S, 1), stride, scale);
}

__global__ void __launch_bounds__(256) gather_rows_kernel(long long nrows, long long len, const long long* __restrict__ idx,
                                                          const double* __restrict__ src, long long ld, double* __restrict__ dst) {
  for (long long r = blockIdx.y; r < nrows; r += gridDim.y) {
    const long long sr = idx[r];
    const double* in = src + (sr < 0 ? 0 : sr) * ld;
    double* out = dst + r * len;
    for (long long c = (long long)blockIdx.x * blockDim.x + threadIdx.x; c < len; c += (long long)gridDim.x * blockDim.x)
      out[c] = sr < 0 ? 0.0 : in[c];
  }
}
int dev_gather_rows(int64_t nrows, int64_t len, const int64_t* idx_dev, const double* src, int64_t ld, double* dst) {
  REQUIRE_INIT();
  if (nrows <= 0 || len <= 0) return QEMB_OK;
  return launch("dev_gather_rows", gather_rows_kernel, dim3((unsigned)std::min<int64_t>((len + 255) / 256, 64), (unsigned)std::min<int64_t>(nrows, 65535)), dim3(256), 0, g_stream,
                nrows, len, (const long long*)idx_dev, src, ld, dst);
}
__global__ void __launch_bounds__(256) scale_rows_kernel(long long nrows, long long len, double* __restrict__ x, const double* __restrict__ s) {
  for (long long r = blockIdx.y; r < nrows; r += gridDim.y) {
    const double f = s[r];
    if (f == 1.0) continue;
    double* row = x + r * len;
    for (long long c = (long long)blockIdx.x * blockDim.x + threadIdx.x; c < len; c += (long long)gridDim.x * blockDim.x) row[c] = (f == 0.0) ? 0.0 : row[c] * f;
  }
}
int dev_scale_rows(int64_t nrows, int64_t len, double* x, const double* s) {
  REQUIRE_INIT();
  if (nrows <= 0 || len <= 0) return QEMB_OK;
  return launch("dev_scale_rows", scale_rows_kernel, dim3((unsigned)std::min<int64_t>((len + 255) / 256, 64), (unsigned)std::min<int64_t>(nrows, 65535)), dim3(256), 0, g_stream,
                nrows, len, x, s);
}

__global__ void __launch_bounds__(256) mirror_lower_kernel(long long n, double* __restrict__ A, long long lda) {
  __shared__ double tile[32][33];
  long long t = xcd_logical_block(make_uint3(blockIdx.x, 0, 0), make_uint3(gridDim.x, 1, 1)).x;
  long long tr = (long long)((sqrt(8.0 * (double)t + 1.0) - 1.0) * 0.5);
  while (tr * (tr + 1) / 2 > t) --tr;
  while ((tr + 1) * (tr + 2) / 2 <= t) ++tr;
  const long long tc = t - tr * (tr + 1) / 2;
  const int tx = threadIdx.x & 31, ty = threadIdx.x >> 5;
#pragma unroll
  for (int i = 0; i < 4; ++i) {
    const long long r = tr * 32 + ty + 8 * i, c = tc * 32 + tx;
    tile[ty + 8 * i][tx] = (r < n && c < n) ? A[r * lda + c] : 0.0;
  }
  __syncthreads();
#pragma unroll
  for (int i = 0; i < 4; ++i) {
    const long long r = tc * 32 + ty + 8 * i, c = tr * 32 + tx;
    if (r < n && c < n && r < c) A[r * lda + c] = tile[tx][ty + 8 * i];
  }
}
int dev_mirror_lower(int64_t n, double* A, int64_t lda) {
  REQUIRE_INIT();
  if (n <= 1) return QEMB_OK;
  const long long nt = (n + 31) / 32;
  return launch("dev_mirror_lower", mirror_lower_kernel, dim3((unsigned)(nt * (nt + 1) / 2)), dim3(256), 0, g_stream, n, A, lda);
}

struct LincombK { const double* x[8]; double c[8]; int n; };
__device__ __forceinline__ void lincomb_kernel_body(const uint3 BID, const uint3 GDIM, long long n, LincombK k, double beta, double* __restrict__ out) {
  for (long long t = (long long)BID.x * blockDim.x + threadIdx.x; t < n; t += (long long)GDIM.x * blockDim.x) {
    double acc = (beta != 0.0) ? beta * out[t] : 0.0;
#pragma unroll
    for (int q = 0; q < 8; ++q) if (q < k.n) acc += k.c[q] * k.x[q][t];
    out[t] = acc;
  }
}
__global__ void __launch_bounds__(256) lincomb_kernel(long long n, LincombK k, double beta, double* __restrict__ out) { lincomb_kernel_body(block_id(), grid_dim(), n, k, beta, out); }
static const Groupable<lincomb_kernel_body, 256> reg_lincomb(lincomb_kernel);
int dev_lincomb(int64_t n, int nterms, const double* coef, const double* const* xs, double beta, double* out) {
  REQUIRE_INIT();
  if (n <= 0) return QEMB_OK;
  if (nterms < 0 || nterms > 8) { set_error("dev_lincomb: at most 8 terms"); return QEMB_ERR_ARG; }
  LincombK k{};
  k.n = nterms;
  for (int q = 0; q < nterms; ++q) { k.x[q] = xs[q]; k.c[q] = coef[q]; }
  const long long blocks = std::min<long long>((n + 255) / 256, 256 * 16);
  return launch("dev_lincomb", lincomb_kernel, dim3((unsigned)blocks), dim3(256), 0, g_stream, n, k, beta, out);
}

__device__ __forceinline__ long long pair_idx(long long i, long long j);
__device__ __forceinline__ void unpair_ge(long long p, long long& x, long long& y) {
  x = (long long)((sqrt(8.0 * (double)p + 1.0) - 1.0) * 0.5);
  while (x * (x + 1) / 2 > p) --x;
  while ((x + 1) * (x + 2) / 2 <= p) ++x;
  y = p - x * (x + 1) / 2;
}
__global__ void __launch_bounds__(256) pack_pair_rows_kernel(long long n, long long ncols, const double* __restrict__ in, double* __restrict__ out) {
  const long long np = n * (n + 1) / 2;
  for (long long p = blockIdx.y; p < np; p += gridDim.y) {
    long long x, y; unpair_ge(p, x, y);
    const double* src = in + (x * n + y) * ncols;
    double* dst = out + p * ncols;
    for (long long c = (long long)blockIdx.x * blockDim.x + threadIdx.x; c < ncols; c += (long long)gridDim.x * blockDim.x) dst[c] = src[c];
  }
}
int dev_pack_pair_rows(int64_t n, int64_t ncols, const double* in, double* out) {
  REQUIRE_INIT();
  const long long np = n * (n + 1) / 2;
  if (np <= 0 || ncols <= 0) return QEMB_OK;
  return launch("dev_pack_pair_rows", pack_pair_rows_kernel, dim3((unsigned)std::min<long long>((ncols + 255) / 256, 256), (unsigned)std::min<long long>(np, 65535)), dim3(256), 0, g_stream,
                n, ncols, in, out);
}
__global__ void __launch_bounds__(256) extract_pf_kernel(long long n, const double* __restrict__ Mp, long long p0, long long q0, long long r0, long long s0,
                                                        long long sp, long long sq, long long sr, long long ss, double* __restrict__ out) {
  const long long nrs = sr * ss;
  for (long long pq = blockIdx.x; pq < sp * sq; pq += gridDim.x) {
    const long long p = pq / sq, q = pq - p * sq;
    const double* src = Mp + pair_idx(p0 + p, q0 + q) * n * n + r0 * n + s0;
    double* dst = out + pq * nrs;
    for (long long t = threadIdx.x; t < nrs; t += blockDim.x) {
      const long long r = t / ss, s = t - r * ss;
      dst[t] = src[r * n + s];
    }
  }
}
int dev_extract_pf(int64_t n, const double* Mp, int64_t p0, int64_t q0, int64_t r0, int64_t s0, int64_t sp, int64_t sq, int64_t sr, int64_t ss, double* out) {
  REQUIRE_INIT();
  if (sp <= 0 || sq <= 0 || sr <= 0 || ss <= 0) return QEMB_OK;
  return launch("dev_extract_pf", extract_pf_kernel, dim3((unsigned)std::min<int64_t>(sp * sq, 1 << 20)), dim3(256), 0, g_stream, n, Mp, p0, q0,
                r0, s0, sp, sq, sr, ss, out);
}
__global__ void __launch_bounds__(256) extract_pf_t_kernel(long long n, const double* __restrict__ T, long long x0, long long r0, long long s0, long long c0,
                                                          long long sx, long long sr, long long ss, long long sc, double* __restrict__ out, long long slab) {
  for (long long rs = blockIdx.x; rs < sr * ss; rs += gridDim.x) {
    const long long r = rs / ss, s = rs - r * ss;
    const double* src = T + pair_idx(r0 + r, s0 + s) * slab + c0 * n + x0;
    for (long long t = threadIdx.x; t < sc * sx; t += blockDim.x) {
      const long long c = t / sx, x = t - c * sx;
      out[(x * sr * ss + rs) * sc + c] = src[c * n + x];
    }
  }
}
int dev_extract_pf_t(int64_t n, const double* T, int64_t x0, int64_t r0, int64_t s0, int64_t c0, int64_t sx, int64_t sr, int64_t ss, int64_t sc, double* out, int64_t slab) {
  REQUIRE_INIT();
  if (sx <= 0 || sr <= 0 || ss <= 0 || sc <= 0) return QEMB_OK;
  if (slab <= 0) slab = n * n;
  if (c0 + sc > slab / n) { set_error("dev_extract_pf_t: rows beyond the slab"); return QEMB_ERR_ARG; }
  return launch("dev_extract_pf_t", extract_pf_t_kernel, dim3((unsigned)std::min<int64_t>(sr * ss, 1 << 20)), dim3(256), 0, g_stream, n, T, x0, r0,
                s0, c0, sx, sr, ss, sc, out, slab);
}
__global__ void __launch_bounds__(256) ladder_pack_vvvv_pf_kernel(long long n, long long o, const double* __restrict__ Mp,
                                                                 double* __restrict__ Vp, long long ldp, double* __restrict__ Vm, long long ldm) {
  const long long v = n - o, np = v * (v + 1) / 2, nm = v * (v - 1) / 2, n2 = n * n;
  for (long long ab = blockIdx.x; ab < np; ab += gridDim.x) {
    long long a, b; unpair_ge(ab, a, b);
    double* vp = Vp + ab * ldp;
    double* vm = (a > b) ? Vm + (a * (a - 1) / 2 + b) * ldm : nullptr;
    for (long long cd0 = threadIdx.x; cd0 < ldp; cd0 += 4 * (long long)blockDim.x) {
      double x[4], y[4]; long long cc[4], dd[4]; bool in[4];
#pragma unroll
      for (int u = 0; u < 4; ++u) {
        const long long cd = cd0 + u * (long long)blockDim.x;
        in[u] = cd < np;
        long long c = 0, d = 0;
        if (in[u]) unpair_ge(cd, c, d);
        cc[u] = c; dd[u] = d;
        x[u] = in[u] ? Mp[pair_idx(o + a, o + c) * n2 + (o + b) * n + (o + d)] : 0.0;
        y[u] = in[u] ? Mp[pair_idx(o + b, o + c) * n2 + (o + a) * n + (o + d)] : 0.0;
      }
#pragma unroll
      for (int u = 0; u < 4; ++u) {
        const long long cd = cd0 + u * (long long)blockDim.x;
        if (cd >= ldp) continue;
        if (!in[u]) { vp[cd] = 0.0; continue; }
        vp[cd] = x[u] + y[u];
        if (vm && cc[u] > dd[u]) vm[cc[u] * (cc[u] - 1) / 2 + dd[u]] = x[u] - y[u];
      }
    }
    if (vm) for (long long q = nm + threadIdx.x; q < ldm; q += blockDim.x) vm[q] = 0.0;
  }
}
int dev_ladder_pack_vvvv_pf(int64_t n, int64_t o, const double* Mp, double* Vp, int64_t ldp, double* Vm, int64_t ldm) {
  REQUIRE_INIT();
  const long long v = n - o, np = v * (v + 1) / 2;
  if (np <= 0) return QEMB_OK;
  return launch("dev_ladder_pack_vvvv_pf", ladder_pack_vvvv_pf_kernel, dim3((unsigned)std::min<long long>(np, 1 << 20)), dim3(256), 0, g_stream, n, o, Mp, Vp, ldp, Vm, ldm);
}

__global__ void __launch_bounds__(256) ladder_pack_vvvv_kernel(long long n, long long o, const double* __restrict__ M,
                                                              double* __restrict__ Vp, long long ldp, double* __restrict__ Vm, long long ldm) {
  const long long v = n - o, np = v * (v + 1) / 2;
  for (long long ab = blockIdx.x; ab < np; ab += gridDim.x) {
    long long a, b; unpair_ge(ab, a, b);
    const double* Ma = M + ((o + a) * n) * n * n + (o + b) * n;
    double* vp = Vp + ab * ldp;
    double* vm = (a > b) ? Vm + (a * (a - 1) / 2 + b) * ldm : nullptr;
    for (long long cd = threadIdx.x; cd < ldp; cd += blockDim.x) {
      if (cd >= np) { vp[cd] = 0.0; continue; }
      long long c, d; unpair_ge(cd, c, d);
      const double x = Ma[(o + c) * n * n + (o + d)], y = Ma[(o + d) * n * n + (o + c)];
      vp[cd] = x + y;
      if (vm && c > d) vm[c * (c - 1) / 2 + d] = x - y;
    }
    if (vm) { const long long nm = v * (v - 1) / 2; for (long long q = nm + threadIdx.x; q < ldm; q += blockDim.x) vm[q] = 0.0; }
  }
}
int dev_ladder_pack_vvvv(int64_t n, int64_t o, const double* M, double* Vp, int64_t ldp, double* Vm, int64_t ldm) {
  REQUIRE_INIT();
  const long long v = n - o, np = v * (v + 1) / 2;
  if (np <= 0) return QEMB_OK;
  return launch("dev_ladder_pack_vvvv", ladder_pack_vvvv_kernel, dim3((unsigned)std::min<long long>(np, 1 << 20)), dim3(256), 0, g_stream, n, o, M, Vp, ldp, Vm, ldm);
}
template <int MODE>
__global__ void __launch_bounds__(256) pack_pm_tiled_kernel(long long rows, long long o, long long v, const double* __restrict__ in, double* __restrict__ Op,
                                                            long long ldp, double* __restrict__ Om, long long ldm) {
  __shared__ double tB[32][33];
  const long long np = v * (v + 1) / 2, nm = v * (v - 1) / 2;
  const uint3 LB = xcd_logical_block(block_id(), grid_dim());
  long long tc, td; unpair_ge((long long)LB.x, tc, td);
  const int tx = threadIdx.x & 31, ty = threadIdx.x >> 5;
  const bool diag = (tc == td);
  for (long long r = LB.y; r < rows; r += gridDim.y) {
    const double* t; double* tp = Op + r * ldp; double* tm;
    if (MODE == 1) {
      long long i, j; unpair_ge(r, i, j);
      t = in + (i * o + j) * v * v;
      tm = (i > j) ? Om + (i * (i - 1) / 2 + j) * ldm : nullptr;
    } else {
      t = in + r * v * v; tm = Om + r * ldm;
    }
    double xa[4];
#pragma unroll
    for (int k = 0; k < 4; ++k) {
      const int rr = ty + 8 * k;
      const long long c = tc * 32 + rr, d = td * 32 + tx;
      xa[k] = (c < v && d < v) ? t[c * v + d] : 0.0;
      if (!diag) {
        const long long d2 = td * 32 + rr, c2 = tc * 32 + tx;
        tB[rr][tx] = (d2 < v && c2 < v) ? t[d2 * v + c2] : 0.0;
      } else {
        tB[rr][tx] = xa[k];
      }
    }
    __syncthreads();
#pragma unroll
    for (int k = 0; k < 4; ++k) {
      const int cc = ty + 8 * k;
      const long long c = tc * 32 + cc, d = td * 32 + tx;
      if (c < v && d <= c) {
        const double x = xa[k], y = tB[tx][cc];
        if (MODE == 1) {
          tp[c * (c + 1) / 2 + d] = (c == d) ? 0.25 * (x + y) : 0.5 * (x + y);
          if (tm && c > d) tm[c * (c - 1) / 2 + d] = 0.5 * (x - y);
        } else {
          tp[c * (c + 1) / 2 + d] = x + y;
          if (c > d) tm[c * (c - 1) / 2 + d] = x - y;
        }
      }
    }
    if (LB.x == 0) {
      for (long long q = np + threadIdx.x; q < ldp; q += 256) tp[q] = 0.0;
      if (tm) for (long long q = nm + threadIdx.x; q < ldm; q += 256) tm[q] = 0.0;
    }
    __syncthreads();
  }
}
__device__ __forceinline__ void ladder_pack_tau_kernel_body(const uint3 BID, const uint3 GDIM, long long o, long long v, const double* __restrict__ tau,
                                                             double* __restrict__ Tp, long long ldp, double* __restrict__ Tm, long long ldm) {
  const long long ij = BID.x, np = v * (v + 1) / 2, nm = v * (v - 1) / 2;
  long long i, j; unpair_ge(ij, i, j);
  const double* t = tau + (i * o + j) * v * v;
  double* tp = Tp + ij * ldp;
  double* tm = (i > j) ? Tm + (i * (i - 1) / 2 + j) * ldm : nullptr;
  const long long chunk = (ldp + GDIM.y - 1) / GDIM.y, cd0 = BID.y * chunk, cd1 = (cd0 + chunk < ldp) ? cd0 + chunk : ldp;
  for (long long cd = cd0 + threadIdx.x; cd < cd1; cd += blockDim.x) {
    if (cd >= np) { tp[cd] = 0.0; continue; }
    long long c, d; unpair_ge(cd, c, d);
    const double x = t[c * v + d], y = t[d * v + c];
    tp[cd] = (c == d) ? 0.25 * (x + y) : 0.5 * (x + y);
    if (tm && c > d) tm[c * (c - 1) / 2 + d] = 0.5 * (x - y);
  }
  if (tm && BID.y == 0) for (long long q = nm + threadIdx.x; q < ldm; q += blockDim.x) tm[q] = 0.0;
}
__global__ void __launch_bounds__(256) ladder_pack_tau_kernel(long long o, long long v, const double* __restrict__ tau,
                                                             double* __restrict__ Tp, long long ldp, double* __restrict__ Tm, long long ldm) { ladder_pack_tau_kernel_body(block_id(), grid_dim(), o, v, tau, Tp, ldp, Tm, ldm); }
static const Groupable<ladder_pack_tau_kernel_body, 256> reg_ladder_pack_tau(ladder_pack_tau_kernel);
int dev_ladder_pack_tau(int64_t o, int64_t v, const double* tau, double* Tp, int64_t ldp, double* Tm, int64_t ldm) {
  REQUIRE_INIT();
  const long long npo = o * (o + 1) / 2;
  if (npo <= 0 || v <= 0) return QEMB_OK;
  if (v >= 32) {
    const long long nt = (v + 31) / 32;
    return launch("dev_ladder_pack_tau", pack_pm_tiled_kernel<1>, dim3((unsigned)(nt * (nt + 1) / 2), (unsigned)std::min<long long>(npo, 65535)), dim3(256), 0, g_stream,
                  npo, o, v, tau, Tp, ldp, Tm, ldm);
  }
  const unsigned slices = (unsigned)std::max<long long>(1, std::min<long long>(16, ldp / 2048));
  return launch("dev_ladder_pack_tau", ladder_pack_tau_kernel, dim3((unsigned)npo, slices), dim3(256), 0, g_stream, o, v, tau, Tp, ldp, Tm, ldm);
}
__global__ void __launch_bounds__(256) pack_pm_cols_kernel(long long rows, long long v, const double* __restrict__ in, double* __restrict__ Op, long long ldp,
                                                          double* __restrict__ Om, long long ldm) {
  const long long np = v * (v + 1) / 2, nm = v * (v - 1) / 2;
  for (long long r = blockIdx.x; r < rows; r += gridDim.x) {
    const double* t = in + r * v * v;
    double* tp = Op + r * ldp;
    double* tm = Om + r * ldm;
    for (long long cd = threadIdx.x; cd < ldp; cd += blockDim.x) {
      if (cd >= np) { tp[cd] = 0.0; continue; }
      long long c, d; unpair_ge(cd, c, d);
      const double x = t[c * v + d], y = t[d * v + c];
      tp[cd] = x + y;
      if (c > d) tm[c * (c - 1) / 2 + d] = x - y;
    }
    for (long long q = nm + threadIdx.x; q < ldm; q += blockDim.x) tm[q] = 0.0;
  }
}
int dev_pack_pm_cols(int64_t rows, int64_t v, const double* in, double* Op, int64_t ldp, double* Om, int64_t ldm) {
  REQUIRE_INIT();
  if (rows <= 0 || v <= 0) return QEMB_OK;
  if (v >= 32) {
    const long long nt = (v + 31) / 32;
    return launch("dev_pack_pm_cols", pack_pm_tiled_kernel<0>, dim3((unsigned)(nt * (nt + 1) / 2), (unsigned)std::min<int64_t>(rows, 16384)), dim3(256), 0, g_stream,
                  rows, 0LL, v, in, Op, ldp, Om, ldm);
  }
  return launch("dev_pack_pm_cols", pack_pm_cols_kernel, dim3((unsigned)std::min<int64_t>(rows, 1 << 20)), dim3(256), 0, g_stream, rows, v, in, Op, ldp, Om, ldm);
}
__device__ __forceinline__ void scatter_pm_rows_kernel_body(const uint3 BID, const uint3 GDIM, long long o, long long ncols, const double* __restrict__ Xp, const double* __restrict__ Xm, double* __restrict__ out, const double* __restrict__ add,
                                                            int Sp, long long strideP, int Sm, long long strideM) {
  const long long ij = BID.y;
  long long i, j; unpair_ge(ij, i, j);
  const double* xp = Xp + ij * ncols;
  const double* xm = (i > j) ? Xm + (i * (i - 1) / 2 + j) * ncols : nullptr;
  double* oij = out + (i * o + j) * ncols;
  double* oji = out + (j * o + i) * ncols;
  const double* aij = add ? add + (i * o + j) * ncols : nullptr;
  const double* aji = add ? add + (j * o + i) * ncols : nullptr;
  for (long long c = (long long)BID.x * blockDim.x + threadIdx.x; c < ncols; c += (long long)GDIM.x * blockDim.x) {
    const double p = slab_sum(xp + c, Sp, strideP);
    if (xm) { const double m = slab_sum(xm + c, Sm, strideM); oij[c] = add ? aij[c] + (p + m) : p + m; oji[c] = add ? aji[c] + (p - m) : p - m; }
    else oij[c] = add ? aij[c] + p : p;
  }
}
__global__ void __launch_bounds__(256) scatter_pm_rows_kernel(long long o, long long ncols, const double* __restrict__ Xp, const double* __restrict__ Xm, double* __restrict__ out, const double* __restrict__ add, int Sp, long long strideP, int Sm, long long strideM) { scatter_pm_rows_kernel_body(block_id(), grid_dim(), o, ncols, Xp, Xm, out, add, Sp, strideP, Sm, strideM); }
static const Groupable<scatter_pm_rows_kernel_body, 256> reg_scatter_pm_rows(scatter_pm_rows_kernel);
int dev_scatter_pm_rows(int64_t o, int64_t ncols, const double* Xp, const double* Xm, double* out, const double* add, int Sp, int64_t strideP, int Sm, int64_t strideM) {
  REQUIRE_INIT();
  const long long npo = o * (o + 1) / 2;
  if (npo <= 0 || ncols <= 0) return QEMB_OK;
  if (npo > 65535) { set_error("dev_scatter_pm_rows: too many pairs"); return QEMB_ERR_ARG; }
  return launch("dev_scatter_pm_rows", scatter_pm_rows_kernel, dim3((unsigned)std::min<long long>((ncols + 255) / 256, 64), (unsigned)npo), dim3(256), 0, g_stream, o, ncols, Xp, Xm, out, add, std::max(Sp, 1), strideP, std::max(Sm, 1), strideM);
}
__device__ __forceinline__ void ccsd_finish_t2_kernel_body(const uint3 BID, const uint3 GDIM, long long o, long long v, double* __restrict__ t2n, const double* __restrict__ U,
                                                            const double* __restrict__ OV, const double* __restrict__ eo, const double* __restrict__ ev) {
  __shared__ double tile[32][33];
  const long long ij = BID.y, i = ij / o, j = ij - i * o;
  const long long nt = (v + 31) / 32;
  const long long ta = BID.x / nt, tb = BID.x - ta * nt;
  const int tx = threadIdx.x & 31, ty = threadIdx.x >> 5;
  const double* Uji = U + (j * o + i) * v * v;
#pragma unroll
  for (int k = 0; k < 4; ++k) {
    const int bb = ty + 8 * k;
    const long long b = tb * 32 + bb, a = ta * 32 + tx;
    tile[bb][tx] = (a < v && b < v) ? Uji[b * v + a] : 0.0;
  }
  __syncthreads();
  const double eij = eo[i] + eo[j];
  const long long base = ij * v * v;
#pragma unroll
  for (int k = 0; k < 4; ++k) {
    const int aa = ty + 8 * k;
    const long long a = ta * 32 + aa, b = tb * 32 + tx;
    if (a < v && b < v) {
      const long long idx = base + a * v + b;
      t2n[idx] = (t2n[idx] + OV[idx] + U[idx] + tile[tx][aa]) / (eij - ev[a] - ev[b]);
    }
  }
}
__global__ void __launch_bounds__(256) ccsd_finish_t2_kernel(long long o, long long v, double* __restrict__ t2n, const double* __restrict__ U,
                                                            const double* __restrict__ OV, const double* __restrict__ eo, const double* __restrict__ ev) { ccsd_finish_t2_kernel_body(block_id(), grid_dim(), o, v, t2n, U, OV, eo, ev); }
static const Groupable<ccsd_finish_t2_kernel_body, 256> reg_ccsd_finish_t2(ccsd_finish_t2_kernel);
int dev_ccsd_finish_t2(int64_t o, int64_t v, double* t2n, const double* U, const double* OV, const double* eo, const double* ev) {
  REQUIRE_INIT();
  if (o <= 0 || v <= 0) return QEMB_OK;
  if (o * o > 65535) { set_error("dev_ccsd_finish_t2: too many occupied pairs"); return QEMB_ERR_ARG; }
  const long long nt = (v + 31) / 32;
  return launch("dev_ccsd_finish_t2", ccsd_finish_t2_kernel, dim3((unsigned)(nt * nt), (unsigned)(o * o)), dim3(256), 0, g_stream, o, v, t2n, U, OV, eo, ev);
}
__device__ __forceinline__ void ccsd_finish_t2_rings_kernel_body(const uint3 BID, const uint3 GDIM, long long o, long long v, double* __restrict__ t2n, const double* __restrict__ U,
                                                                   const double* __restrict__ OV, const double* __restrict__ RS, const double* __restrict__ M,
                                                                   const double* __restrict__ eo, const double* __restrict__ ev, double* __restrict__ t1n) {
  __shared__ double tile[32][33];
  const uint3 LB = xcd_logical_block(BID, GDIM);
  long long i, j; unpair_ge((long long)LB.y, i, j);
  const long long nt = (v + 31) / 32;
  const long long ta = LB.x / nt, tb = LB.x - ta * nt;
  const int tx = threadIdx.x & 31, ty = threadIdx.x >> 5;
  const long long vv = v * v, ov = o * v;
  const double* Uij = U + (i * o + j) * vv;
  const double* Uji = U + (j * o + i) * vv;
  const double* RSij = RS + i * v * ov + j * v;
  const double* RSji = RS + j * v * ov + i * v;
  const double* Mij = M + i * v * ov + j * v;
  const double* Mji = M + j * v * ov + i * v;
#pragma unroll
  for (int k = 0; k < 4; ++k) {
    const int bb = ty + 8 * k;
    const long long b = tb * 32 + bb, a = ta * 32 + tx;
    tile[bb][tx] = (a < v && b < v) ? ((Uji[b * v + a] + RSji[b * ov + a]) - 0.5 * Mji[b * ov + a]) - Mij[b * ov + a] : 0.0;
  }
  __syncthreads();
  const double eij = eo[i] + eo[j];
  double res[4];
#pragma unroll
  for (int k = 0; k < 4; ++k) {
    const int aa = ty + 8 * k;
    const long long a = ta * 32 + aa, b = tb * 32 + tx;
    res[k] = 0.0;
    if (a < v && b < v) {
      const long long idx = (i * o + j) * vv + a * v + b;
      const double straight = ((Uij[a * v + b] + RSij[a * ov + b]) - 0.5 * Mij[a * ov + b]) - Mji[a * ov + b];
      res[k] = (t2n[idx] + OV[idx] + straight + tile[tx][aa]) / (eij - ev[a] - ev[b]);
      t2n[idx] = res[k];
    }
  }
  if (i != j) {
    __syncthreads();
#pragma unroll
    for (int k = 0; k < 4; ++k) tile[ty + 8 * k][tx] = res[k];
    __syncthreads();
#pragma unroll
    for (int k = 0; k < 4; ++k) {
      const int bb = ty + 8 * k;
      const long long b = tb * 32 + bb, a = ta * 32 + tx;
      if (a < v && b < v) t2n[(j * o + i) * vv + b * v + a] = tile[tx][bb];
    }
  }
  if (t1n && LB.x == 0 && LB.y == 0)
    for (long long t = threadIdx.x; t < ov; t += blockDim.x) t1n[t] /= eo[t / v] - ev[t % v];
}
__global__ void __launch_bounds__(256) ccsd_finish_t2_rings_kernel(long long o, long long v, double* __restrict__ t2n, const double* __restrict__ U, const double* __restrict__ OV,
                                                                  const double* __restrict__ RS, const double* __restrict__ M, const double* __restrict__ eo,
                                                                  const double* __restrict__ ev, double* __restrict__ t1n) {
  ccsd_finish_t2_rings_kernel_body(block_id(), grid_dim(), o, v, t2n, U, OV, RS, M, eo, ev, t1n);
}
static const Groupable<ccsd_finish_t2_rings_kernel_body, 256> reg_ccsd_finish_t2_rings(ccsd_finish_t2_rings_kernel);
int dev_ccsd_finish_t2_rings(int64_t o, int64_t v, double* t2n, const double* U, const double* OV, const double* RS, const double* M, const double* eo, const double* ev, double* t1n) {
  REQUIRE_INIT();
  if (o <= 0 || v <= 0) return QEMB_OK;
  const long long npo = o * (o + 1) / 2, nt = (v + 31) / 32;
  if (npo > 65535) { set_error("dev_ccsd_finish_t2_rings: too many occupied pairs"); return QEMB_ERR_ARG; }
  return launch("dev_ccsd_finish_t2_rings", ccsd_finish_t2_rings_kernel, dim3((unsigned)(nt * nt), (unsigned)npo), dim3(256), 0, g_stream, o, v, t2n, U, OV, RS, M, eo, ev, t1n);
}
__device__ __forceinline__ void ladder_scatter_pm_kernel_body(const uint3 BID, const uint3 GDIM, long long o, long long v, const double* __restrict__ Rp, long long ldp,
                                                               const double* __restrict__ Rm, long long ldm, double* __restrict__ t2,
                                                               const double* __restrict__ Hp, const double* __restrict__ Hm, int assign,
                                                               int Sp, long long strideP, int Sm, long long strideM, long long ldhp, long long ldhm) {
  __shared__ double sp[32][33], sm[32][33];
  const uint3 LB = xcd_logical_block(BID, GDIM);
  const long long ij = LB.y;
  long long i, j; unpair_ge(ij, i, j);
  long long t = LB.x, ta, tb; unpair_ge(t, ta, tb);
  const int tx = threadIdx.x & 31, ty = threadIdx.x >> 5;
  const double* rp = Rp + ij * ldp;
  const double* rm = (i > j) ? Rm + (i * (i - 1) / 2 + j) * ldm : nullptr;
  const double* hp = Hp ? Hp + ij * ldhp : nullptr;
  const double* hm = (Hm && i > j) ? Hm + (i * (i - 1) / 2 + j) * ldhm : nullptr;
  double* tij = t2 + (i * o + j) * v * v;
  double* tji = t2 + (j * o + i) * v * v;
#pragma unroll
  for (int k = 0; k < 4; ++k) {
    const int aa = ty + 8 * k;
    const long long a = ta * 32 + aa, b = tb * 32 + tx;
    double p = 0.0, m = 0.0;
    if (a < v && b <= a) {
      p = slab_sum(rp + a * (a + 1) / 2 + b, Sp, strideP);
      if (hp) p += (a == b ? 2.0 : 1.0) * hp[a * (a + 1) / 2 + b];
      if (rm && b < a) { m = slab_sum(rm + a * (a - 1) / 2 + b, Sm, strideM); if (hm) m += hm[a * (a - 1) / 2 + b]; }
// ... 1197 lines not shown
```

Baseline: 57.04.

## Build MO integral blocks directly from packed DF pair product without full unpack

When neither Vl nor T34 intermediates are needed, the DF AO2MO path now extracts every MO integral block, including a packed ovvv and the vvvv ladder packs, straight from the packed pair-product matrix. This skips unpacking the full n^4 tensor. The three-quarter transformed blocks come from a GEMM over only the ov pair columns instead of all pairs. The ovvv plus/minus packing gains a tiled kernel mode that reads ovvv in its natural layout, removing a perm4 transpose and a temporary buffer. The cost is several new gather kernels with strided, irregular reads and more code paths to keep correct.

```diff
diff --git a/include/qemb_hip_ops.h b/include/qemb_hip_ops.h
--- a/include/qemb_hip_ops.h
+++ b/include/qemb_hip_ops.h
@@ -94,6 +94,16 @@
 int qemb_op_extract_pf_t(int64_t n, const double* T, int64_t x0, int64_t r0, int64_t s0, int64_t c0, int64_t sx, int64_t sr,
                          int64_t ss, int64_t sc, double* out);
 int qemb_op_ladder_pack_vvvv_pf(int64_t n, int64_t o, const double* Mp, double* Vp, int64_t ldp, double* Vm, int64_t ldm);
+int qemb_op_extract_pf_t_compact(int64_t n, const double* T, int64_t x0, int64_t c0, int64_t sx, int64_t sr, int64_t ss, int64_t sc,
+                                 double* out, int64_t slab);
+int qemb_op_gather_pair_cols(int64_t rows, int64_t n, const double* in, int64_t r0, int64_t s0, int64_t sr, int64_t ss, double* out);
+int qemb_op_extract_ps(int64_t n, const double* S, int64_t p0, int64_t q0, int64_t r0, int64_t s0, int64_t sp, int64_t sq,
+                       int64_t sr, int64_t ss, double* out);
+int qemb_op_extract_ps_packed(int64_t n, const double* S, int64_t p0, int64_t q0, int64_t r0, int64_t sp, int64_t sq, int64_t sr, double* out);
+int qemb_op_unpack_pair_block(int64_t n, int64_t o, const double* S, double* Mv, int64_t ld);
+int qemb_op_ladder_pack_vvvv_pf_ld(int64_t n, int64_t o, const double* Mp, int64_t ld, double* Vp, int64_t ldp, double* Vm, int64_t ldm);
+int qemb_op_pack_pm_ovvv(int64_t o, int64_t v, const double* ovvv, double* Op, int64_t ldp, double* Om, int64_t ldm);
+int qemb_op_df_pair_product(int64_t np, int64_t naux, const double* bb, double* out);
 int qemb_op_unpack_tril_rows(int64_t rows, int64_t n, const double* packed, double* full);
 int qemb_op_pack_tril_rows(int64_t rows, int64_t n, const double* full, double* packed);
 int qemb_op_jacobi_eigh(int64_t n, double* A, double* w, double* V, int* sweeps);
diff --git a/quemb_amd/_lib.py b/quemb_amd/_lib.py
--- a/quemb_amd/_lib.py
+++ b/quemb_amd/_lib.py
@@ -133,6 +133,14 @@
     f("qemb_op_extract_pf", I, L, P, L, L, L, L, L, L, L, L, P)
     f("qemb_op_extract_pf_t", I, L, P, L, L, L, L, L, L, L, L, P)
     f("qemb_op_ladder_pack_vvvv_pf", I, L, L, P, P, L, P, L)
+    f("qemb_op_extract_pf_t_compact", I, L, P, L, L, L, L, L, L, P, L)
+    f("qemb_op_gather_pair_cols", I, L, L, P, L, L, L, L, P)
+    f("qemb_op_extract_ps", I, L, P, L, L, L, L, L, L, L, L, P)
+    f("qemb_op_extract_ps_packed", I, L, P, L, L, L, L, L, L, P)
+    f("qemb_op_unpack_pair_block", I, L, L, P, P, L)
+    f("qemb_op_ladder_pack_vvvv_pf_ld", I, L, L, P, L, P, L, P, L)
+    f("qemb_op_pack_pm_ovvv", I, L, L, P, P, L, P, L)
+    f("qemb_op_df_pair_product", I, L, L, P, P)
     f("qemb_op_pack_tril_rows", I, L, L, P, P)
     f("qemb_op_jacobi_eigh", I, L, P, P, P, C.POINTER(I))
     f("qemb_op_scf_fused_max", I)
diff --git a/quemb_amd/csrc/api.cpp b/quemb_amd/csrc/api.cpp
--- a/quemb_amd/csrc/api.cpp
+++ b/quemb_amd/csrc/api.cpp
@@ -237,6 +237,24 @@
   return dev_extract_pf_t(n, T, x0, r0, s0, c0, sx, sr, ss, sc, out);
 }
 int qemb_op_ladder_pack_vvvv_pf(int64_t n, int64_t o, const double* Mp, double* Vp, int64_t ldp, double* Vm, int64_t ldm) { return dev_ladder_pack_vvvv_pf(n, o, Mp, Vp, ldp, Vm, ldm); }
+int qemb_op_extract_pf_t_compact(int64_t n, const double* T, int64_t x0, int64_t c0, int64_t sx, int64_t sr, int64_t ss, int64_t sc, double* out, int64_t slab) {
+  return dev_extract_pf_t_compact(n, T, x0, c0, sx, sr, ss, sc, out, slab);
+}
+int qemb_op_gather_pair_cols(int64_t rows, int64_t n, const double* in, int64_t r0, int64_t s0, int64_t sr, int64_t ss, double* out) {
+  return dev_gather_pair_cols(rows, n, in, r0, s0, sr, ss, out);
+}
+int qemb_op_extract_ps(int64_t n, const double* S, int64_t p0, int64_t q0, int64_t r0, int64_t s0, int64_t sp, int64_t sq, int64_t sr, int64_t ss, double* out) {
+  return dev_extract_ps(n, S, p0, q0, r0, s0, sp, sq, sr, ss, out);
+}
+int qemb_op_extract_ps_packed(int64_t n, const double* S, int64_t p0, int64_t q0, int64_t r0, int64_t sp, int64_t sq, int64_t sr, double* out) {
+  return dev_extract_ps_packed(n, S, p0, q0, r0, sp, sq, sr, out);
+}
+int qemb_op_unpack_pair_block(int64_t n, int64_t o, const double* S, double* Mv, int64_t ld) { return dev_unpack_pair_block(n, o, S, Mv, ld); }
+int qemb_op_ladder_pack_vvvv_pf_ld(int64_t n, int64_t o, const double* Mp, int64_t ld, double* Vp, int64_t ldp, double* Vm, int64_t ldm) {
+  return dev_ladder_pack_vvvv_pf_ld(n, o, Mp, ld, Vp, ldp, Vm, ldm);
+}
+int qemb_op_pack_pm_ovvv(int64_t o, int64_t v, const double* ovvv, double* Op, int64_t ldp, double* Om, int64_t ldm) { return dev_pack_pm_ovvv(o, v, ovvv, Op, ldp, Om, ldm); }
+int qemb_op_df_pair_product(int64_t np, int64_t naux, const double* bb, double* out) { return df_pair_product(np, naux, bb, out); }
 int qemb_op_unpack_tril_pair_rows(int64_t nr, int64_t n, const double* in, double* full) { return dev_unpack_tril_pair_rows(nr, n, in, full); }
 int qemb_op_unpack_tril_rows(int64_t rows, int64_t n, const double* p, double* f) { return dev_unpack_tril_rows(rows, n, p, f); }
 int qemb_op_pack_tril_rows(int64_t rows, int64_t n, const double* f, double* p) { return dev_pack_tril_rows(rows, n, f, p); }
diff --git a/quemb_amd/csrc/ccsd.cpp b/quemb_amd/csrc/ccsd.cpp
--- a/quemb_amd/csrc/ccsd.cpp
+++ b/quemb_amd/csrc/ccsd.cpp
@@ -24,6 +24,42 @@
     QTRY(dev_extract_pf_t(n, T, o, 0, o, 0, v, o, v, nf, out.A1, slab));
     QTRY(dev_extract_pf_t(n, T, 0, 0, o, 0, o, o, v, nf, out.A2, slab));
   }
+  return 0;
+}
+
+static int mo_three_quarter_blocks_ov(int n, int o, int nf, const double* T, int64_t slab, MoIntegrals& out) {
+  const int v = n - o;
+  QTRY(out.A1.alloc((int64_t)v * o * v * nf));
+  QTRY(out.A2.alloc((int64_t)o * o * v * nf));
+  QTRY(dev_extract_pf_t_compact(n, T, o, 0, v, o, v, nf, out.A1, slab));
+  QTRY(dev_extract_pf_t_compact(n, T, 0, 0, o, o, v, nf, out.A2, slab));
+  return 0;
+}
+
+static int mo_blocks_from_pair_product(int n, int o, const double* S, double* work, MoIntegrals& out) {
+  const int v = n - o;
+  const int64_t npv = (int64_t)v * (v + 1) / 2, nm = (int64_t)v * (v - 1) / 2;
+  QTRY(out.oooo.alloc((int64_t)o * o * o * o));
+  QTRY(out.ovoo.alloc((int64_t)o * v * o * o));
+  QTRY(out.ovov.alloc((int64_t)o * v * o * v));
+  QTRY(out.oovv.alloc((int64_t)o * o * v * v));
+  QTRY(out.ovvo.alloc((int64_t)o * v * v * o));
+  QTRY(out.ovvv.alloc((int64_t)o * v * v * v));
+  QTRY(out.ovvv_pk.alloc((int64_t)o * v * npv));
+  QTRY(dev_extract_ps(n, S, 0, 0, 0, 0, o, o, o, o, out.oooo));
+  QTRY(dev_extract_ps(n, S, 0, o, 0, 0, o, v, o, o, out.ovoo));
+  QTRY(dev_extract_ps(n, S, 0, o, 0, o, o, v, o, v, out.ovov));
+  QTRY(dev_extract_ps(n, S, 0, 0, o, o, o, o, v, v, out.oovv));
+  QTRY(dev_extract_ps(n, S, 0, o, o, 0, o, v, v, o, out.ovvo));
+  QTRY(dev_extract_ps_packed(n, S, 0, o, o, o, v, v, out.ovvv_pk));
+  QTRY(dev_unpack_tril_rows((int64_t)o * v, v, out.ovvv_pk, out.ovvv));
+  out.ldp = npv + (npv & 1); out.ldm = nm + (nm & 1);
+  if (out.ldm == 0) out.ldm = 2;
+  QTRY(out.Vp.alloc(npv * out.ldp));
+  QTRY(out.Vm.alloc(std::max<int64_t>(nm, 1) * out.ldm));
+  const int64_t ldv = mo_slab_ld(v);
+  QTRY(dev_unpack_pair_block(n, o, S, work, ldv));
+  QTRY(dev_ladder_pack_vvvv_pf_ld(v, 0, work, ldv, out.Vp, out.ldp, out.Vm, out.ldm));
   return 0;
 }
 
@@ -106,6 +142,19 @@
   QTRY(dev_pack_tril_rows(naux, n, Lu, Lpk));
   Lu.release();
   QTRY(df_pair_product(np, naux, Lpk, X1));
+  if (!build_Vl && !build_T34) {
+    if (nf > 0) {
+      DBuf Lov;
+      QTRY(Lov.alloc((int64_t)naux * o * v));
+      QTRY(dev_gather_pair_cols(naux, n, Lpk, 0, o, o, v, Lov));
+      QTRY(gemm((int64_t)o * v, (int64_t)nf * n, naux, 1.0, Lov, (int64_t)o * v, false, Lh, n2, false, 0.0, X0, (int64_t)nf * n));
+      QTRY(mo_three_quarter_blocks_ov(n, o, nf, X0, (int64_t)nf * n, out));
+    }
+    Lh.release(); Lpk.release();
+    QTRY(mo_blocks_from_pair_product(n, o, X1, X0, out));
+    QTRY(lap_AO2MO.close());
+    return 0;
+  }
   QTRY(dev_unpack_tril_rows(np, n, X1, X0));
   if (nf > 0) {
     QTRY(gemm(np, (int64_t)nf * n, naux, 1.0, Lpk, np, false, Lh, n2, false, 0.0, X1, (int64_t)nf * n));
@@ -147,16 +196,20 @@
   QTRY(dcopy(N2, W2base_, Lph1_));
   QTRY(axpby(N2, 2.0, W1base_, -1.0, Lph1_));
   {
-    DBuf OVl;
-    QTRY(OVl.alloc(o * v * vv));
-    QTRY(perm4(OVl, I_.ovvv, o, v, v, v, 0, 2, 3, 1));
     QTRY(OVp_.alloc(nov * I_.ldp)); QTRY(OVm_.alloc(nov * I_.ldm));
-    QTRY(dev_pack_pm_cols(nov, v, OVl, OVp_, I_.ldp, OVm_, I_.ldm));
+    if (v >= 32) QTRY(dev_pack_pm_ovvv(o, v, I_.ovvv, OVp_, I_.ldp, OVm_, I_.ldm));
+    else {
+      DBuf OVl;
+      QTRY(OVl.alloc(o * v * vv));
+      QTRY(perm4(OVl, I_.ovvv, o, v, v, v, 0, 2, 3, 1));
+      QTRY(dev_pack_pm_cols(nov, v, OVl, OVp_, I_.ldp, OVm_, I_.ldm));
+    }
   }
   {
     const int64_t npv = v * (v + 1) / 2;
-    QTRY(ovvv_pk_.alloc(o * v * npv)); QTRY(ZCp_.alloc(oo * npv));
-    QTRY(dev_pack_tril_rows(o * v, v, I_.ovvv, ovvv_pk_));
+    QTRY(ZCp_.alloc(oo * npv));
+    if (I_.ovvv_pk.p) ovvv_pk_ = std::move(I_.ovvv_pk);
+    else { QTRY(ovvv_pk_.alloc(o * v * npv)); QTRY(dev_pack_tril_rows(o * v, v, I_.ovvv, ovvv_pk_)); }
   }
   QTRY(Gp_.alloc(oo * I_.ldp)); QTRY(Gm_.alloc(oo * I_.ldm));
   QTRY(dev_pack_pm_cols(oo, v, OVoovv_, Gp_, I_.ldp, Gm_, I_.ldm));
diff --git a/quemb_amd/csrc/ccsd.h b/quemb_amd/csrc/ccsd.h
--- a/quemb_amd/csrc/ccsd.h
+++ b/quemb_amd/csrc/ccsd.h
@@ -17,6 +17,7 @@
 struct MoIntegrals {
   int n = 0, o = 0, v = 0, nf = 0;
   DBuf oooo, ovoo, ovov, oovv, ovvo, ovvv;
+  DBuf ovvv_pk;
   DBuf Vl;
   DBuf Vp, Vm;
   int64_t ldp = 0, ldm = 0;
diff --git a/quemb_amd/csrc/dev_ops.h b/quemb_amd/csrc/dev_ops.h
--- a/quemb_amd/csrc/dev_ops.h
+++ b/quemb_amd/csrc/dev_ops.h
@@ -136,10 +136,17 @@
 int dev_extract_pf_t(int64_t n, const double* T, int64_t x0, int64_t r0, int64_t s0, int64_t c0, int64_t sx, int64_t sr,
                      int64_t ss, int64_t sc, double* out, int64_t slab = 0);
 int dev_ladder_pack_vvvv_pf(int64_t n, int64_t o, const double* Mp, double* Vp, int64_t ldp, double* Vm, int64_t ldm);
+int dev_extract_pf_t_compact(int64_t n, const double* T, int64_t x0, int64_t c0, int64_t sx, int64_t sr, int64_t ss, int64_t sc, double* out, int64_t slab = 0);
+int dev_gather_pair_cols(int64_t rows, int64_t n, const double* in, int64_t r0, int64_t s0, int64_t sr, int64_t ss, double* out);
+int dev_extract_ps(int64_t n, const double* S, int64_t p0, int64_t q0, int64_t r0, int64_t s0, int64_t sp, int64_t sq, int64_t sr, int64_t ss, double* out);
+int dev_extract_ps_packed(int64_t n, const double* S, int64_t p0, int64_t q0, int64_t r0, int64_t sp, int64_t sq, int64_t sr, double* out);
+int dev_unpack_pair_block(int64_t n, int64_t o, const double* S, double* Mv, int64_t ld);
+int dev_ladder_pack_vvvv_pf_ld(int64_t n, int64_t o, const double* Mp, int64_t ld, double* Vp, int64_t ldp, double* Vm, int64_t ldm);
 
 int dev_ladder_pack_vvvv(int64_t n, int64_t o, const double* M, double* Vp, int64_t ldp, double* Vm, int64_t ldm);
 int dev_ladder_pack_tau(int64_t o, int64_t v, const double* tau, double* Tp, int64_t ldp, double* Tm, int64_t ldm);
 int dev_pack_pm_cols(int64_t rows, int64_t v, const double* in, double* Op, int64_t ldp, double* Om, int64_t ldm);
+int dev_pack_pm_ovvv(int64_t o, int64_t v, const double* ovvv, double* Op, int64_t ldp, double* Om, int64_t ldm);
 int dev_scatter_pm_rows(int64_t o, int64_t ncols, const double* Xp, const double* Xm, double* out, const double* add = nullptr, int Sp = 1, int64_t strideP = 0,
                         int Sm = 1, int64_t strideM = 0);
 int dev_ccsd_finish_t2(int64_t o, int64_t v, double* t2n, const double* U, const double* OV, const double* eo, const double* ev);
diff --git a/quemb_amd/csrc/dev_ops_hip.hip b/quemb_amd/csrc/dev_ops_hip.hip
--- a/quemb_amd/csrc/dev_ops_hip.hip
+++ b/quemb_amd/csrc/dev_ops_hip.hip
@@ -1400,10 +1400,11 @@
                 r0, s0, sp, sq, sr, ss, out);
 }
 __global__ void __launch_bounds__(256) extract_pf_t_kernel(long long n, const double* __restrict__ T, long long x0, long long r0, long long s0, long long c0,
-                                                          long long sx, long long sr, long long ss, long long sc, double* __restrict__ out, long long slab) {
+                                                          long long sx, long long sr, long long ss, long long sc, double* __restrict__ out, long long slab,
+                                                          int compact) {
   for (long long rs = blockIdx.x; rs < sr * ss; rs += gridDim.x) {
     const long long r = rs / ss, s = rs - r * ss;
-    const double* src = T + pair_idx(r0 + r, s0 + s) * slab + c0 * n + x0;
+    const double* src = T + (compact ? rs : pair_idx(r0 + r, s0 + s)) * slab + c0 * n + x0;
     for (long long t = threadIdx.x; t < sc * sx; t += blockDim.x) {
       const long long c = t / sx, x = t - c * sx;
       out[(x * sr * ss + rs) * sc + c] = src[c * n + x];
@@ -1416,11 +1417,121 @@
   if (slab <= 0) slab = n * n;
   if (c0 + sc > slab / n) { set_error("dev_extract_pf_t: rows beyond the slab"); return QEMB_ERR_ARG; }
   return launch("dev_extract_pf_t", extract_pf_t_kernel, dim3((unsigned)std::min<int64_t>(sr * ss, 1 << 20)), dim3(256), 0, g_stream, n, T, x0, r0,
-                s0, c0, sx, sr, ss, sc, out, slab);
-}
-__global__ void __launch_bounds__(256) ladder_pack_vvvv_pf_kernel(long long n, long long o, const double* __restrict__ Mp,
+                s0, c0, sx, sr, ss, sc, out, slab, 0);
+}
+int dev_extract_pf_t_compact(int64_t n, const double* T, int64_t x0, int64_t c0, int64_t sx, int64_t sr, int64_t ss, int64_t sc, double* out, int64_t slab) {
+  REQUIRE_INIT();
+  if (sx <= 0 || sr <= 0 || ss <= 0 || sc <= 0) return QEMB_OK;
+  if (slab <= 0) slab = n * n;
+  if (c0 + sc > slab / n || x0 + sx > n) { set_error("dev_extract_pf_t_compact: rows beyond the slab"); return QEMB_ERR_ARG; }
+  return launch("dev_extract_pf_t_compact", extract_pf_t_kernel, dim3((unsigned)std::min<int64_t>(sr * ss, 1 << 20)), dim3(256), 0, g_stream, n, T, x0,
+                (long long)0, (long long)0, c0, sx, sr, ss, sc, out, slab, 1);
+}
+__global__ void __launch_bounds__(256) gather_pair_cols_kernel(long long rows, long long np, const double* __restrict__ in, long long r0, long long s0,
+                                                              long long sr, long long ss, double* __restrict__ out) {
+  const long long nc = sr * ss;
+  for (long long L = blockIdx.y; L < rows; L += gridDim.y)
+    for (long long t = (long long)blockIdx.x * blockDim.x + threadIdx.x; t < nc; t += (long long)gridDim.x * blockDim.x) {
+      const long long r = t / ss, s = t - r * ss;
+      out[L * nc + t] = in[L * np + pair_idx(r0 + r, s0 + s)];
+    }
+}
+int dev_gather_pair_cols(int64_t rows, int64_t n, const double* in, int64_t r0, int64_t s0, int64_t sr, int64_t ss, double* out) {
+  REQUIRE_INIT();
+  if (rows <= 0 || sr <= 0 || ss <= 0) return QEMB_OK;
+  if (r0 < 0 || s0 < 0 || r0 + sr > n || s0 + ss > n) { set_error("dev_gather_pair_cols: pairs beyond n"); return QEMB_ERR_ARG; }
+  return launch("dev_gather_pair_cols", gather_pair_cols_kernel, dim3((unsigned)std::min<int64_t>((sr * ss + 255) / 256, 1024), (unsigned)std::min<int64_t>(rows, 65535)),
+                dim3(256), 0, g_stream, rows, n * (n + 1) / 2, in, r0, s0, sr, ss, out);
+}
+__global__ void __launch_bounds__(256) extract_ps_kernel(long long np, const double* __restrict__ S, long long p0, long long q0, long long r0, long long s0,
+                                                        long long sp, long long sq, long long sr, long long ss, double* __restrict__ out) {
+  const long long nrs = sr * ss;
+  for (long long pq = blockIdx.x; pq < sp * sq; pq += gridDim.x) {
+    const long long p = pq / sq, q = pq - p * sq;
+    const double* src = S + pair_idx(p0 + p, q0 + q) * np;
+    double* dst = out + pq * nrs;
+    for (long long t = threadIdx.x; t < nrs; t += blockDim.x) {
+      const long long r = t / ss, s = t - r * ss;
+      dst[t] = src[pair_idx(r0 + r, s0 + s)];
+    }
+  }
+}
+int dev_extract_ps(int64_t n, const double* S, int64_t p0, int64_t q0, int64_t r0, int64_t s0, int64_t sp, int64_t sq, int64_t sr, int64_t ss, double* out) {
+  REQUIRE_INIT();
+  if (sp <= 0 || sq <= 0 || sr <= 0 || ss <= 0) return QEMB_OK;
+  if (p0 < 0 || q0 < 0 || r0 < 0 || s0 < 0 || p0 + sp > n || q0 + sq > n || r0 + sr > n || s0 + ss > n) { set_error("dev_extract_ps: block beyond n"); return QEMB_ERR_ARG; }
+  return launch("dev_extract_ps", extract_ps_kernel, dim3((unsigned)std::min<int64_t>(sp * sq, 1 << 20)), dim3(256), 0, g_stream, n * (n + 1) / 2, S, p0, q0,
+                r0, s0, sp, sq, sr, ss, out);
+}
+__global__ void __launch_bounds__(256) extract_ps_packed_kernel(long long np, const double* __restrict__ S, long long p0, long long q0, long long r0,
+                                                               long long sp, long long sq, long long sr, double* __restrict__ out) {
+  const long long npr = sr * (sr + 1) / 2;
+  const int lane = threadIdx.x & 63, wave = threadIdx.x >> 6;
+  for (long long pq = blockIdx.x; pq < sp * sq; pq += gridDim.x) {
+    const long long p = pq / sq, q = pq - p * sq;
+    const double* src = S + pair_idx(p0 + p, q0 + q) * np;
+    double* dst = out + pq * npr;
+    for (long long r = wave; r < sr; r += 4) {
+      const double* run = src + (r0 + r) * (r0 + r + 1) / 2 + r0;
+      double* o = dst + r * (r + 1) / 2;
+      for (long long s = lane; s <= r; s += 64) o[s] = run[s];
+    }
+  }
+}
+int dev_extract_ps_packed(int64_t n, const double* S, int64_t p0, int64_t q0, int64_t r0, int64_t sp, int64_t sq, int64_t sr, double* out) {
+  REQUIRE_INIT();
+  if (sp <= 0 || sq <= 0 || sr <= 0) return QEMB_OK;
+  if (p0 < 0 || q0 < 0 || r0 < 0 || p0 + sp > n || q0 + sq > n || r0 + sr > n) { set_error("dev_extract_ps_packed: block beyond n"); return QEMB_ERR_ARG; }
+  return launch("dev_extract_ps_packed", extract_ps_packed_kernel, dim3((unsigned)std::min<int64_t>(sp * sq, 1 << 20)), dim3(256), 0, g_stream, n * (n + 1) / 2, S,
+                p0, q0, r0, sp, sq, sr, out);
+}
+__global__ void __launch_bounds__(256) unpack_pair_block_kernel(long long n, long long o, const double* __restrict__ S, double* __restrict__ Mv, long long ld) {
+  __shared__ double tile[32][33];
+  const long long v = n - o, npn = n * (n + 1) / 2, npv = v * (v + 1) / 2, slab = v * ld;
+  const int tx = threadIdx.x & 31, ty = threadIdx.x >> 5;
+  const uint3 LB = xcd_logical_block(block_id(), grid_dim());
+  long long tk, tl; unpair_ge((long long)LB.x, tk, tl);
+  for (long long r = LB.y; r < npv; r += gridDim.y) {
+    long long a, c; unpair_ge(r, a, c);
+    const double* src = S + pair_idx(o + a, o + c) * npn;
+    double* dst = Mv + r * slab;
+    double xr[4];
+#pragma unroll
+    for (int i = 0; i < 4; ++i) {
+      const int kk = ty + 8 * i;
+      const long long k = tk * 32 + kk, l = tl * 32 + tx;
+      xr[i] = (k < v && l <= k) ? src[(o + k) * (o + k + 1) / 2 + o + l] : 0.0;
+      tile[kk][tx] = xr[i];
+    }
+#pragma unroll
+    for (int i = 0; i < 4; ++i) {
+      const int kk = ty + 8 * i;
+      const long long k = tk * 32 + kk, l = tl * 32 + tx;
+      if (k < v && l <= k) dst[k * ld + l] = xr[i];
+    }
+    __syncthreads();
+#pragma unroll
+    for (int i = 0; i < 4; ++i) {
+      const int kk = ty + 8 * i;
+      const long long lr = tl * 32 + kk, kc = tk * 32 + tx;
+      if (kc < v && lr < kc) dst[lr * ld + kc] = tile[tx][kk];
+    }
+    __syncthreads();
+  }
+}
+static int64_t unpack_walkers(int64_t rows, int64_t ntiles);
+int dev_unpack_pair_block(int64_t n, int64_t o, const double* S, double* Mv, int64_t ld) {
+  REQUIRE_INIT();
+  const int64_t v = n - o, npv = v * (v + 1) / 2;
+  if (npv <= 0) return QEMB_OK;
+  if (o < 0 || ld < v) { set_error("dev_unpack_pair_block: need 0 <= o < n and ld >= n - o"); return QEMB_ERR_ARG; }
+  const int64_t nt = (v + 31) / 32;
+  return launch("dev_unpack_pair_block", unpack_pair_block_kernel, dim3((unsigned)(nt * (nt + 1) / 2), (unsigned)unpack_walkers(npv, nt * (nt + 1) / 2)), dim3(256), 0, g_stream,
+                n, o, S, Mv, ld);
+}
+__global__ void __launch_bounds__(256) ladder_pack_vvvv_pf_kernel(long long n, long long o, const double* __restrict__ Mp, long long ld,
                                                                  double* __restrict__ Vp, long long ldp, double* __restrict__ Vm, long long ldm) {
-  const long long v = n - o, np = v * (v + 1) / 2, nm = v * (v - 1) / 2, n2 = n * n;
+  const long long v = n - o, np = v * (v + 1) / 2, nm = v * (v - 1) / 2, n2 = n * ld;
   for (long long ab = blockIdx.x; ab < np; ab += gridDim.x) {
     long long a, b; unpair_ge(ab, a, b);
     double* vp = Vp + ab * ldp;
@@ -1434,8 +1545,8 @@
         long long c = 0, d = 0;
         if (in[u]) unpair_ge(cd, c, d);
         cc[u] = c; dd[u] = d;
-        x[u] = in[u] ? Mp[pair_idx(o + a, o + c) * n2 + (o + b) * n + (o + d)] : 0.0;
-        y[u] = in[u] ? Mp[pair_idx(o + b, o + c) * n2 + (o + a) * n + (o + d)] : 0.0;
+        x[u] = in[u] ? Mp[pair_idx(o + a, o + c) * n2 + (o + b) * ld + (o + d)] : 0.0;
+        y[u] = in[u] ? Mp[pair_idx(o + b, o + c) * n2 + (o + a) * ld + (o + d)] : 0.0;
       }
 #pragma unroll
       for (int u = 0; u < 4; ++u) {
@@ -1449,12 +1560,14 @@
     if (vm) for (long long q = nm + threadIdx.x; q < ldm; q += blockDim.x) vm[q] = 0.0;
   }
 }
-int dev_ladder_pack_vvvv_pf(int64_t n, int64_t o, const double* Mp, double* Vp, int64_t ldp, double* Vm, int64_t ldm) {
+int dev_ladder_pack_vvvv_pf_ld(int64_t n, int64_t o, const double* Mp, int64_t ld, double* Vp, int64_t ldp, double* Vm, int64_t ldm) {
   REQUIRE_INIT();
   const long long v = n - o, np = v * (v + 1) / 2;
   if (np <= 0) return QEMB_OK;
-  return launch("dev_ladder_pack_vvvv_pf", ladder_pack_vvvv_pf_kernel, dim3((unsigned)std::min<long long>(np, 1 << 20)), dim3(256), 0, g_stream, n, o, Mp, Vp, ldp, Vm, ldm);
-}
+  if (ld < n) { set_error("dev_ladder_pack_vvvv_pf_ld: ld < n"); return QEMB_ERR_ARG; }
+  return launch("dev_ladder_pack_vvvv_pf", ladder_pack_vvvv_pf_kernel, dim3((unsigned)std::min<long long>(np, 1 << 20)), dim3(256), 0, g_stream, n, o, Mp, (long long)ld, Vp, ldp, Vm, ldm);
+}
+int dev_ladder_pack_vvvv_pf(int64_t n, int64_t o, const double* Mp, double* Vp, int64_t ldp, double* Vm, int64_t ldm) { return dev_ladder_pack_vvvv_pf_ld(n, o, Mp, n, Vp, ldp, Vm, ldm); }
 
 __global__ void __launch_bounds__(256) ladder_pack_vvvv_kernel(long long n, long long o, const double* __restrict__ M,
                                                               double* __restrict__ Vp, long long ldp, double* __restrict__ Vm, long long ldm) {
@@ -1495,18 +1608,22 @@
       long long i, j; unpair_ge(r, i, j);
       t = in + (i * o + j) * v * v;
       tm = (i > j) ? Om + (i * (i - 1) / 2 + j) * ldm : nullptr;
+    } else if (MODE == 2) {
+      const long long k = r / v, a = r - k * v;
+      t = in + k * v * v * v + a * v; tm = Om + r * ldm;
     } else {
       t = in + r * v * v; tm = Om + r * ldm;
     }
+    const long long rs = (MODE == 2) ? v * v : v;
     double xa[4];
 #pragma unroll
     for (int k = 0; k < 4; ++k) {
       const int rr = ty + 8 * k;
       const long long c = tc * 32 + rr, d = td * 32 + tx;
-      xa[k] = (c < v && d < v) ? t[c * v + d] : 0.0;
+      xa[k] = (c < v && d < v) ? t[c * rs + d] : 0.0;
       if (!diag) {
         const long long d2 = td * 32 + rr, c2 = tc * 32 + tx;
-        tB[rr][tx] = (d2 < v && c2 < v) ? t[d2 * v + c2] : 0.0;
+        tB[rr][tx] = (d2 < v && c2 < v) ? t[d2 * rs + c2] : 0.0;
       } else {
         tB[rr][tx] = xa[k];
       }
@@ -1517,7 +1634,7 @@
       const int cc = ty + 8 * k;
       const long long c = tc * 32 + cc, d = td * 32 + tx;
       if (c < v && d <= c) {
-        const double x = xa[k], y = tB[tx][cc];
+        const double x = (MODE == 2) ? tB[tx][cc] : xa[k], y = (MODE == 2) ? xa[k] : tB[tx][cc];
         if (MODE == 1) {
           tp[c * (c + 1) / 2 + d] = (c == d) ? 0.25 * (x + y) : 0.5 * (x + y);
           if (tm && c > d) tm[c * (c - 1) / 2 + d] = 0.5 * (x - y);
@@ -1592,6 +1709,14 @@
                   rows, 0LL, v, in, Op, ldp, Om, ldm);
   }
   return launch("dev_pack_pm_cols", pack_pm_cols_kernel, dim3((unsigned)std::min<int64_t>(rows, 1 << 20)), dim3(256), 0, g_stream, rows, v, in, Op, ldp, Om, ldm);
+}
+int dev_pack_pm_ovvv(int64_t o, int64_t v, const double* ovvv, double* Op, int64_t ldp, double* Om, int64_t ldm) {
+  REQUIRE_INIT();
+  if (o <= 0 || v <= 0) return QEMB_OK;
+  if (v < 32) { set_error("dev_pack_pm_ovvv: tiled pass only (v >= 32)"); return QEMB_ERR_ARG; }
+  const long long nt = (v + 31) / 32;
+  return launch("dev_pack_pm_ovvv", pack_pm_tiled_kernel<2>, dim3((unsigned)(nt * (nt + 1) / 2), (unsigned)std::min<int64_t>(o * v, 16384)), dim3(256), 0, g_stream,
+                o * v, 0LL, v, ovvv, Op, ldp, Om, ldm);
 }
 __device__ __forceinline__ void scatter_pm_rows_kernel_body(const uint3 BID, const uint3 GDIM, long long o, long long ncols, const double* __restrict__ Xp, const double* __restrict__ Xm, double* __restrict__ out, const double* __restrict__ add,
                                                             int Sp, long long strideP, int Sm, long long strideM) {
diff --git a/quemb_amd/csrc/mo_blocks_ops_hostcheck.cpp b/quemb_amd/csrc/mo_blocks_ops_hostcheck.cpp
--- /dev/null
+++ b/quemb_amd/csrc/mo_blocks_ops_hostcheck.cpp
@@ -0,0 +1,66 @@
+#ifdef QEMB_HOSTCHECK
+#include <algorithm>
+#include "dev_ops.h"
+
+namespace qemb {
+
+static inline int64_t pidx(int64_t i, int64_t j) { return i >= j ? i * (i + 1) / 2 + j : j * (j + 1) / 2 + i; }
+
+int dev_extract_pf_t_compact(int64_t n, const double* T, int64_t x0, int64_t c0, int64_t sx, int64_t sr, int64_t ss, int64_t sc, double* out, int64_t slab) {
+  if (slab <= 0) slab = n * n;
+  for (int64_t x = 0; x < sx; ++x) for (int64_t r = 0; r < sr; ++r) for (int64_t s = 0; s < ss; ++s) for (int64_t c = 0; c < sc; ++c)
+    out[((x * sr + r) * ss + s) * sc + c] = T[(r * ss + s) * slab + (c0 + c) * n + (x0 + x)];
+  return 0;
+}
+int dev_gather_pair_cols(int64_t rows, int64_t n, const double* in, int64_t r0, int64_t s0, int64_t sr, int64_t ss, double* out) {
+  const int64_t np = n * (n + 1) / 2;
+  for (int64_t L = 0; L < rows; ++L) for (int64_t r = 0; r < sr; ++r) for (int64_t s = 0; s < ss; ++s) out[(L * sr + r) * ss + s] = in[L * np + pidx(r0 + r, s0 + s)];
+  return 0;
+}
+int dev_extract_ps(int64_t n, const double* S, int64_t p0, int64_t q0, int64_t r0, int64_t s0, int64_t sp, int64_t sq, int64_t sr, int64_t ss, double* out) {
+  const int64_t np = n * (n + 1) / 2;
+  for (int64_t p = 0; p < sp; ++p) for (int64_t q = 0; q < sq; ++q) for (int64_t r = 0; r < sr; ++r) for (int64_t s = 0; s < ss; ++s)
+    out[((p * sq + q) * sr + r) * ss + s] = S[pidx(p0 + p, q0 + q) * np + pidx(r0 + r, s0 + s)];
+  return 0;
+}
+int dev_extract_ps_packed(int64_t n, const double* S, int64_t p0, int64_t q0, int64_t r0, int64_t sp, int64_t sq, int64_t sr, double* out) {
+  const int64_t np = n * (n + 1) / 2, npr = sr * (sr + 1) / 2;
+  for (int64_t p = 0; p < sp; ++p) for (int64_t q = 0; q < sq; ++q) for (int64_t r = 0; r < sr; ++r) for (int64_t s = 0; s <= r; ++s)
+    out[(p * sq + q) * npr + pidx(r, s)] = S[pidx(p0 + p, q0 + q) * np + pidx(r0 + r, r0 + s)];
+  return 0;
+}
+int dev_unpack_pair_block(int64_t n, int64_t o, const double* S, double* Mv, int64_t ld) {
+  const int64_t v = n - o, np = n * (n + 1) / 2;
+  for (int64_t a = 0; a < v; ++a) for (int64_t c = 0; c <= a; ++c) for (int64_t b = 0; b < v; ++b) for (int64_t d = 0; d < v; ++d)
+    Mv[(pidx(a, c) * v + b) * ld + d] = S[pidx(o + a, o + c) * np + pidx(o + b, o + d)];
+  return 0;
+}
+int dev_ladder_pack_vvvv_pf_ld(int64_t n, int64_t o, const double* Mp, int64_t ld, double* Vp, int64_t ldp, double* Vm, int64_t ldm) {
+  const int64_t v = n - o;
+  for (int64_t a = 0; a < v; ++a) for (int64_t b = 0; b <= a; ++b) {
+    double* vp = Vp + (a * (a + 1) / 2 + b) * ldp; std::fill(vp, vp + ldp, 0.0);
+    double* vm = a > b ? Vm + (a * (a - 1) / 2 + b) * ldm : nullptr; if (vm) std::fill(vm, vm + ldm, 0.0);
+    for (int64_t c = 0; c < v; ++c) for (int64_t d = 0; d <= c; ++d) {
+      const double x = Mp[(pidx(o + a, o + c) * n + (o + b)) * ld + (o + d)], y = Mp[(pidx(o + b, o + c) * n + (o + a)) * ld + (o + d)];
+      vp[c * (c + 1) / 2 + d] = x + y;
+      if (vm && c > d) vm[c * (c - 1) / 2 + d] = x - y;
+    }
+  }
+  return 0;
+}
+int dev_pack_pm_ovvv(int64_t o, int64_t v, const double* in, double* Op, int64_t ldp, double* Om, int64_t ldm) {
+  if (v < 32) { set_error("dev_pack_pm_ovvv: tiled pass only (v >= 32)"); return QEMB_ERR_ARG; }
+  for (int64_t k = 0; k < o; ++k) for (int64_t a = 0; a < v; ++a) {
+    double* tp = Op + (k * v + a) * ldp; std::fill(tp, tp + ldp, 0.0);
+    double* tm = Om + (k * v + a) * ldm; std::fill(tm, tm + ldm, 0.0);
+    for (int64_t c = 0; c < v; ++c) for (int64_t d = 0; d <= c; ++d) {
+      const double x = in[((k * v + d) * v + a) * v + c], y = in[((k * v + c) * v + a) * v + d];
+      tp[c * (c + 1) / 2 + d] = x + y;
+      if (c > d) tm[c * (c - 1) / 2 + d] = x - y;
+    }
+  }
+  return 0;
+}
+
+}
+#endif
```

Result: faster. 57.65 (median of 6 runs) (+1.1%).
